# CPJKU/beat_this

Measured on AMD Instinct MI355X. Metric: audio-seconds processed/sec, higher is better.
Workload: dtype f32 activations, f16x3 products (3 x f16 MFMA on hi+lo operand halves, f32 accumulate); main-layer attention P.V: 2 x, probabilities as fp16 hi parts

## Files before the change

beat_this_amd/_lib.py:

```python
from __future__ import annotations

import ctypes as C
import os
import subprocess

import torch

PKG_DIR = os.path.dirname(os.path.abspath(__file__))
LIB_PATH = os.path.join(PKG_DIR, "libbeat_this_amd.so")
if os.environ.get("BT_DEV") == "1" and os.environ.get("BT_LIB_PATH"):
    LIB_PATH = os.environ["BT_LIB_PATH"]
SOURCES = ["gemm.hip", "gemm2.hip", "gemm3.hip", "gemm_mx8.hip", "attn.hip", "attn2.hip", "fused.hip", "fused2.hip", "qkv_front.hip", "frontend.hip", "logmel.hip",
           "tail.hip", "dbn.hip", "metrics.hip", "loss.hip", "data.hip", "train.hip", "optim.hip", "engine.hip"]
HEADERS = ["common.h", "chain.h", "kernels.h", "dropout.h", "train_mixed.inc", "attn_x3_loop.inc", "attn_hq2_loop.inc", os.path.join("..", "..", "include", "beat_this_amd.h")]

BT_OK, BT_ERR_ARG, BT_ERR_HIP, BT_ERR_WORKSPACE = 0, -1, -2, -3
ABI_VERSION = 600
PREC_F32, PREC_HALF, PREC_F32X3 = 0, 1, 3
OPT_X3_ATTN_P16, OPT_X3_GEMM_FP8, OPT_WS_GUARD = 1, 2, 3
MAX_LAYERS = 32
PROFILE_CATEGORIES = ["stem", "qkv_gemm", "attn_flash", "out_gemm", "ff1_gemm", "ff2_gemm", "conv_gemm",
                      "linear_gemm", "head", "ff_fused", "attn_freq_fused", "layer_tail"]

GEMM_EPI_STORE, GEMM_EPI_RESID, GEMM_EPI_QKV = 0, 1, 2
# ... 92 lines not shown
                ("residual", C.c_int32), ("sum_head", C.c_int32), ("reserved", C.c_int32), ("rope", C.c_void_p),
                ("gamma", C.c_void_p), ("w1", C.c_void_p), ("b1", C.c_void_p), ("w2", C.c_void_p), ("b2", C.c_void_p),
                ("w3", C.c_void_p), ("x", C.c_void_p), ("y", C.c_void_p), ("y2", C.c_void_p), ("save_o", C.c_void_p),
                ("save_lse", C.c_void_p), ("gy", C.c_void_p), ("gy2", C.c_void_p), ("gx", C.c_void_p), ("g_gamma", C.c_void_p),
                ("g_w1", C.c_void_p), ("g_b1", C.c_void_p), ("g_w2", C.c_void_p), ("g_b2", C.c_void_p), ("g_w3", C.c_void_p),
                ("ws", C.c_void_p), ("ws_bytes", C.c_size_t)]


class TrainDropout(C.Structure):
    _fields_ = [("p", C.c_float), ("reserved", C.c_uint32), ("seed", C.c_uint64), ("stream", C.c_uint64)]


class OptimTensor(C.Structure):
    _fields_ = [("param", C.c_void_p), ("offset", C.c_int64), ("numel", C.c_int64), ("group", C.c_int32), ("reserved", C.c_int32)]


class OptimChunk(C.Structure):
    _fields_ = [("tensor", C.c_int32), ("chunk", C.c_int32)]


class OptimGroup(C.Structure):
    _fields_ = [("decay", C.c_float), ("one_minus_beta1", C.c_float), ("beta2", C.c_float), ("one_minus_beta2", C.c_float),
                ("step_size", C.c_float), ("bias2_sqrt", C.c_float), ("eps", C.c_float), ("reserved", C.c_float)]


OPTIM_MAX_GROUPS = 8


class OptimHyper(C.Structure):
    _fields_ = [("n_groups", C.c_int32), ("zero_grads", C.c_int32), ("grad_scale", C.c_float), ("reserved", C.c_int32),
                ("g", OptimGroup * OPTIM_MAX_GROUPS)]


G3_FF1, G3_RESID, G3_QKV = 0, 1, 2
UNIT_STEM, UNIT_PARTIAL, UNIT_CONV, UNIT_LINEAR, UNIT_ATTN, UNIT_FF, UNIT_NORM, UNIT_FRONT_ATTN, UNIT_FRONT_FF = range(9)
TRAIN_UNIT_HEAD = 16
TRAIN_DW_ROWS, TRAIN_CS_ROWS, TRAIN_ATTN_BLOCK = 1024, 64, 64
DROP_ATTN_P, DROP_ATTN_OUT, DROP_FF_HIDDEN, DROP_FF_OUT = range(4)
OPTIM_CHUNK, OPTIM_NORM_SLICE = 4096, 4096

EXPORTS = {
    "bt_last_error": (C.c_char_p, []),
    "bt_version": (C.c_int, []),
    "bt_half_is_bf16": (C.c_int, []),
    "bt_struct_sizes": (None, [C.POINTER(C.c_int32)]),
    "bt_engine_create": (C.c_int, [C.POINTER(ModelDesc), C.POINTER(C.c_void_p)]),
    "bt_engine_destroy": (None, [C.c_void_p]),
    "bt_engine_set_option": (C.c_int, [C.c_void_p, C.c_int, C.c_int]),
    "bt_engine_get_option": (C.c_int, [C.c_void_p, C.c_int, C.POINTER(C.c_int)]),
    "bt_workspace_bytes": (C.c_size_t, [C.c_void_p, C.c_int, C.c_int, C.c_int]),
    "bt_workspace_regions": (C.c_int, [C.c_void_p, C.c_int, C.c_int, C.c_int, C.POINTER(C.c_int64), C.c_int]),
    "bt_forward": (C.c_int, [C.c_void_p, C.c_void_p, C.c_int, C.c_void_p, C.c_int, C.c_int, C.c_void_p, C.c_size_t,
                             C.c_void_p, C.c_void_p]),
    "bt_forward_stages": (C.c_int, [C.c_void_p, C.c_void_p, C.c_int, C.c_int, C.c_int, C.c_void_p, C.c_int, C.c_int, C.c_void_p,
                                    C.c_size_t, C.c_void_p, C.c_void_p, C.c_void_p]),
    "bt_forward_unit": (C.c_int, [C.c_void_p, C.c_void_p, C.c_int, C.c_int, C.c_int, C.c_void_p, C.c_void_p, C.c_int, C.c_int,
                                  C.c_void_p, C.c_size_t]),
    "bt_split_chunks": (C.c_int, [C.c_void_p, C.c_void_p, C.c_int64, C.c_void_p, C.c_int, C.c_int, C.c_void_p]),
    "bt_aggregate": (C.c_int, [C.c_void_p, C.c_void_p, C.c_void_p, C.c_void_p, C.c_int, C.c_int, C.c_int, C.c_int64,
                               C.c_void_p, C.c_void_p]),
    "bt_logmel": (C.c_int, [C.c_void_p, C.POINTER(LogmelTables), C.c_void_p, C.c_int64, C.c_void_p]),
    "bt_resample": (C.c_int, [C.c_void_p, C.c_void_p, C.c_int64, C.c_int, C.c_int, C.c_void_p, C.c_int, C.c_void_p,
                              C.c_int64]),
    "bt_peaks": (C.c_int, [C.c_void_p, C.c_void_p, C.c_int64, C.c_int, C.c_void_p, C.c_void_p]),
    "bt_deduplicate_peaks_host": (C.c_int, [C.c_void_p, C.c_int, C.c_double, C.c_void_p, C.POINTER(C.c_int32)]),
    "bt_postprocess_host": (C.c_int, [C.c_void_p, C.c_int, C.c_void_p, C.c_int, C.c_double, C.c_void_p,
                                      C.POINTER(C.c_int32), C.c_void_p, C.POINTER(C.c_int32)]),
    "bt_audio2beats_plan": (C.c_int, [C.c_void_p, C.c_int64, C.c_int, C.c_int, C.c_int, C.POINTER(A2BPlan)]),
    "bt_audio2beats_enqueue": (C.c_int, [C.c_void_p, C.c_void_p, C.c_int, C.POINTER(LogmelTables), C.c_void_p, C.c_int64, C.c_int, C.c_int,
                                         C.c_void_p, C.c_int, C.c_void_p, C.c_size_t, C.c_void_p, C.c_int]),
    "bt_profile_begin": (None, [C.c_void_p]),
    "bt_profile_end": (C.c_int, [C.c_void_p, C.c_void_p, C.c_void_p, C.c_int]),
    "bt_resample_batch": (C.c_int, [C.c_void_p, C.c_void_p, C.c_int, C.c_int64, C.c_int, C.c_int, C.c_void_p, C.c_int,
                                    C.c_void_p]),
    "bt_logmel_batch": (C.c_int, [C.c_void_p, C.POINTER(LogmelTables), C.c_void_p, C.c_int, C.c_int64, C.c_void_p]),
    "bt_split_chunks_batch": (C.c_int, [C.c_void_p, C.c_void_p, C.c_void_p, C.c_int, C.c_int, C.c_void_p]),
    "bt_aggregate_batch": (C.c_int, [C.c_void_p, C.c_void_p, C.c_void_p, C.c_void_p, C.c_void_p, C.c_int, C.c_int64,
                                     C.c_int, C.c_int, C.c_void_p, C.c_void_p]),
    "bt_peaks_batch": (C.c_int, [C.c_void_p, C.c_void_p, C.c_void_p, C.c_int, C.c_void_p, C.c_void_p]),
    "bt_peaks_host": (C.c_int, [C.c_void_p, C.c_int64, C.c_void_p, C.POINTER(C.c_int32)]),
    "bt_gemm": (C.c_int, [C.c_void_p, C.c_int, C.POINTER(GemmArgs)]),
    "bt_attention": (C.c_int, [C.c_void_p, C.c_int, C.POINTER(AttnArgs)]),
    "bt_gemm3": (C.c_int, [C.c_void_p, C.POINTER(Gemm3Args)]),
    "bt_gemm_mx8": (C.c_int, [C.c_void_p, C.c_void_p, C.c_void_p, C.c_void_p, C.c_void_p, C.c_void_p, C.c_int, C.c_int, C.c_int, C.c_int64]),
    "bt_attn_frag_blocks": (C.c_int, [C.c_int]),
    "bt_attention_frag": (C.c_int, [C.c_void_p, C.POINTER(AttnFragArgs)]),
    "bt_qkv_front": (C.c_int, [C.c_void_p, C.c_int, C.POINTER(PairWeights), C.c_void_p, C.c_void_p, C.c_int, C.c_int, C.c_int,
                               C.c_void_p, C.c_void_p, C.c_void_p, C.c_void_p, C.c_int]),
    "bt_outff_fused": (C.c_int, [C.c_void_p, C.c_int, C.POINTER(PairWeights), C.c_void_p, C.c_void_p, C.c_int64, C.c_void_p]),
    "bt_attnff_fused": (C.c_int, [C.c_void_p, C.c_int, C.POINTER(PairWeights), C.c_void_p, C.c_void_p, C.c_int64]),
    "bt_layer_tail": (C.c_int, [C.c_void_p, C.POINTER(PairWeights), C.c_int, C.c_void_p, C.c_void_p, C.c_int64, C.c_void_p,
                                C.c_void_p]),
    "bt_ff_fused": (C.c_int, [C.c_void_p, C.c_int, C.POINTER(PairWeights), C.c_void_p, C.c_int64]),
    "bt_dbn_tables": (C.c_int, [C.c_double, C.c_double, C.c_double, C.c_int, C.c_double, C.c_double, C.c_double, C.c_void_p,
                                C.c_int, C.c_void_p, C.POINTER(C.c_size_t)]),
    "bt_dbn_workspace_bytes": (C.c_size_t, [C.c_void_p, C.c_int, C.c_int64]),
    "bt_dbn_decode": (C.c_int, [C.c_void_p, C.c_void_p, C.c_void_p, C.c_void_p, C.c_int, C.c_void_p, C.c_int, C.c_int64,
                                C.c_void_p, C.c_void_p, C.c_size_t]),
    "bt_dbn_viterbi": (C.c_int, [C.c_void_p, C.c_void_p, C.c_void_p, C.c_int, C.c_void_p, C.c_int64, C.c_void_p, C.c_void_p,
                                 C.c_void_p, C.c_size_t]),
    "bt_dbn_viterbi_host": (C.c_int, [C.c_void_p, C.c_int, C.c_void_p, C.c_int64, C.c_void_p, C.c_void_p]),
    "bt_dbn_host": (C.c_int, [C.c_void_p, C.c_void_p, C.c_void_p, C.c_int64, C.c_void_p, C.POINTER(C.c_int32)]),
    "bt_dbn_host_act": (C.c_int, [C.c_void_p, C.c_void_p, C.c_int64, C.c_void_p, C.POINTER(C.c_int32)]),
    "bt_beat_metrics_workspace_bytes": (C.c_size_t, [C.c_int, C.c_int64, C.c_int64]),
    "bt_beat_metrics": (C.c_int, [C.c_void_p, C.c_void_p, C.c_void_p, C.c_void_p, C.c_void_p, C.c_int, C.c_double, C.c_double,
                                  C.c_double, C.c_double, C.c_double, C.c_void_p, C.c_size_t, C.c_void_p]),
    "bt_beat_metrics_host": (C.c_int, [C.c_void_p, C.c_void_p, C.c_void_p, C.c_void_p, C.c_int, C.c_double, C.c_double,
                                       C.c_double, C.c_double, C.c_double, C.c_void_p]),
    "bt_bce_loss_workspace_bytes": (C.c_size_t, [C.c_int, C.c_int64]),
    "bt_bce_loss": (C.c_int, [C.c_void_p, C.c_int, C.c_int, C.c_float, C.c_void_p, C.c_void_p, C.c_int, C.c_void_p, C.c_int,
                              C.c_void_p, C.c_int, C.c_void_p, C.c_int, C.c_int64, C.c_int64, C.c_void_p, C.c_size_t,
                              C.c_void_p, C.c_void_p, C.c_void_p, C.c_int, C.c_void_p, C.c_void_p]),
    "bt_bce_loss_backward": (C.c_int, [C.c_void_p, C.c_void_p, C.c_int64, C.c_void_p, C.c_int, C.c_int64, C.c_void_p, C.c_int]),
    "bt_bce_loss_host": (C.c_int, [C.c_int, C.c_int, C.c_float, C.c_void_p, C.c_int, C.c_void_p, C.c_int, C.c_void_p, C.c_int,
                                   C.c_void_p, C.c_int, C.c_void_p, C.c_void_p, C.c_void_p, C.c_void_p, C.c_void_p]),
    "bt_train_batch_struct_sizes": (None, [C.POINTER(C.c_int32)]),
    "bt_train_batch": (C.c_int, [C.c_void_p, C.c_void_p, C.c_int, C.c_int64, C.c_void_p, C.c_int, C.c_int, C.c_void_p, C.c_int,
                                 C.c_void_p, C.c_int, C.c_void_p, C.c_void_p, C.c_int64, C.c_double, C.c_void_p, C.c_int,
                                 C.c_void_p, C.c_void_p, C.c_void_p, C.c_void_p]),
    "bt_train_batch_host": (C.c_int, [C.c_void_p, C.c_int, C.c_int64, C.c_void_p, C.c_int, C.c_int, C.c_void_p, C.c_int,
                                      C.c_void_p, C.c_int, C.c_void_p, C.c_void_p, C.c_int64, C.c_double, C.c_void_p, C.c_int,
                                      C.c_void_p, C.c_void_p, C.c_void_p, C.c_void_p]),
    "bt_train_struct_sizes": (None, [C.POINTER(C.c_int32)]),
    "bt_train_workspace_bytes": (C.c_size_t, [C.c_int, C.c_int, C.c_int, C.c_int, C.c_int, C.c_int]),
    "bt_train_forward": (C.c_int, [C.c_void_p, C.c_int, C.POINTER(TrainArgs)]),
    "bt_train_backward": (C.c_int, [C.c_void_p, C.c_int, C.POINTER(TrainArgs)]),
    "bt_train_dropout_struct_sizes": (None, [C.POINTER(C.c_int32)]),
    "bt_train_workspace_bytes_dropout": (C.c_size_t, [C.c_int, C.c_int, C.c_int, C.c_int, C.c_int, C.c_int]),
    "bt_train_forward_dropout": (C.c_int, [C.c_void_p, C.c_int, C.POINTER(TrainArgs), C.POINTER(TrainDropout)]),
    "bt_train_backward_dropout": (C.c_int, [C.c_void_p, C.c_int, C.POINTER(TrainArgs), C.POINTER(TrainDropout)]),
    "bt_philox4x32_10_host": (None, [C.POINTER(C.c_uint32), C.POINTER(C.c_uint32), C.POINTER(C.c_uint32)]),
    "bt_dropout_mask_host": (C.c_int, [C.POINTER(TrainDropout), C.c_int, C.c_int, C.c_int, C.c_int, C.c_int, C.c_void_p]),
    "bt_train_workspace_bytes_mixed": (C.c_size_t, [C.c_int, C.c_int, C.c_int, C.c_int, C.c_int, C.c_int, C.c_int]),
    "bt_train_forward_mixed": (C.c_int, [C.c_void_p, C.c_int, C.POINTER(TrainArgs), C.POINTER(TrainDropout)]),
    "bt_train_backward_mixed": (C.c_int, [C.c_void_p, C.c_int, C.POINTER(TrainArgs), C.POINTER(TrainDropout)]),
    "bt_train_matmul_mixed": (C.c_int, [C.c_void_p, C.c_int, C.c_void_p, C.c_void_p, C.c_int, C.c_int, C.c_int, C.c_void_p]),
# ... 149 lines not shown
```

beat_this_amd/csrc/attn2.hip:

```cpp
#include <cstdlib>

#include "common.h"
#include "kernels.h"

namespace {

constexpr int KB = 4;
constexpr int BLK_BYTES = 2048;
constexpr int TILE_BYTES = KB * BLK_BYTES;
constexpr int SMEM_BYTES = 2 * 2 * TILE_BYTES + 16;

typedef const __attribute__((address_space(1))) void* gptr_t;
typedef __attribute__((address_space(3))) void* lptr_t;

DEVI int lane_id_fresh() {
  int z;
  asm volatile("s_mov_b32 %0, 0" : "=s"(z));
  return __builtin_amdgcn_mbcnt_hi(~0u, __builtin_amdgcn_mbcnt_lo(~0u, z));
}
DEVI unsigned pk2(float a, float b) {
  const hfx2 t = {(hf)a, (hf)b};
  return __builtin_bit_cast(unsigned, t);
}
DEVI void zero16(f32x16& a) {
// ... 905 lines not shown
template <int OUT>
DEVI void store_rows_x(const AttnFragP& p, const QStateX& st, float l_tot, int qi, bool okq, int sh, int g, float& amax) {
  const int seq = sh / p.heads, head = sh - seq * p.heads;
  const float gatev = okq ? p.gates[(long)sh * p.nbp * 32 + qi] : 0.f;
  const long orow = okq ? (long)(seq / p.o_div) * p.o_outer + (long)(seq % p.o_div) * p.o_inner + (long)qi * p.o_tok : 0;
  const float scale = okq ? gatev / l_tot : 0.f;
  if constexpr (OUT == 1) {
    float* op = reinterpret_cast<float*>(p.out) + orow * p.inner + head * 32 + 4 * g;
    if (okq) {
#pragma unroll
      for (int a = 0; a < 4; ++a)
        *reinterpret_cast<f32x4*>(op + 8 * a) = f32x4{st.acc[4 * a] * scale, st.acc[4 * a + 1] * scale,
                                                       st.acc[4 * a + 2] * scale, st.acc[4 * a + 3] * scale};
    }
  } else {
    hf* op = reinterpret_cast<hf*>(p.out) + orow * 2 * p.inner + head * 64 + 8 * g;
#pragma unroll
    for (int k = 0; k < 2; ++k) {
      unsigned xh[2], xl[2], yh[2], yl[2];
#pragma unroll
      for (int i = 0; i < 2; ++i) {
        const float a0 = st.acc[8 * k + 2 * i] * scale, a1 = st.acc[8 * k + 2 * i + 1] * scale;
        const float b0 = st.acc[8 * k + 4 + 2 * i] * scale, b1 = st.acc[8 * k + 4 + 2 * i + 1] * scale;
        split_hl4(a0, a1, b0, b1, xh[i], xl[i], yh[i], yl[i]);
        amax = fmaxf(amax, fmaxf(fmaxf(fabsf(a0), fabsf(a1)), fmaxf(fabsf(b0), fabsf(b1))));
        const float nan_probe = (a0 + a1) + (b0 + b1);
        amax = (okq && nan_probe != nan_probe) ? __builtin_inff() : amax;
      }
      auto h0 = __builtin_amdgcn_permlane32_swap(xh[0], yh[0], false, false);
      auto h1 = __builtin_amdgcn_permlane32_swap(xh[1], yh[1], false, false);
      if (p.out_f32 == 2) {
        const float s0 = st.acc[8 * k] * scale, s1 = st.acc[8 * k + 1] * scale, s2 = st.acc[8 * k + 2] * scale, s3 = st.acc[8 * k + 3] * scale;
        const float t0 = st.acc[8 * k + 4] * scale, t1 = st.acc[8 * k + 5] * scale, t2 = st.acc[8 * k + 6] * scale, t3 = st.acc[8 * k + 7] * scale;
        auto b8 = __builtin_amdgcn_permlane32_swap(pk4_f8(s0, s1, s2, s3), pk4_f8(t0, t1, t2, t3), false, false);
        auto c8 = __builtin_amdgcn_permlane32_swap(lo4_f8(s0, s1, s2, s3, xh[0], xh[1]), lo4_f8(t0, t1, t2, t3, yh[0], yh[1]), false, false);
        if (okq) {
          *reinterpret_cast<u32x4*>(op + 16 * k) = u32x4{h0[0], h1[0], h0[1], h1[1]};
          char* gb = reinterpret_cast<char*>(op) - 16 * g;
          *reinterpret_cast<u32x2*>(gb + 64 + 16 * k + 8 * g) = u32x2{b8[0], b8[1]};
          *reinterpret_cast<u32x2*>(gb + 96 + 16 * k + 8 * g) = u32x2{c8[0], c8[1]};
        }
      } else {
      auto l0 = __builtin_amdgcn_permlane32_swap(xl[0], yl[0], false, false);
      auto l1 = __builtin_amdgcn_permlane32_swap(xl[1], yl[1], false, false);
      if (okq) {
        *reinterpret_cast<u32x4*>(op + 16 * k) = u32x4{h0[0], h1[0], h0[1], h1[1]};
        *reinterpret_cast<u32x4*>(op + 32 + 16 * k) = u32x4{l0[0], l1[0], l0[1], l1[1]};
      }
      }
    }
  }
}

template <int QB, int OUT, int KBX, int MINW, bool P16>
__global__ __launch_bounds__(256, MINW) void attn_frag_x3_kernel(const AttnFragP p, int nqt, int sh_total) {
  constexpr int TILEX_BYTES = KBX * BLKX_BYTES;
  __shared__ __attribute__((aligned(16))) char smem[2 * 2 * TILEX_BYTES + 16];
  const int bid = blockIdx.x;
  const int idx = bid >> 3;
  const int sh = (idx / nqt) * 8 + (bid & 7);
  const int qt = idx % nqt;
  if (sh >= sh_total) return;
  const int tid = threadIdx.x, lane = tid & 63, wave = __builtin_amdgcn_readfirstlane(tid >> 6);
  const int g = lane >> 5, lr = lane & 31;
  const int L = p.L;
  const int nblk = (L + 31) >> 5;
  const long seq_off = (long)sh * p.nbp * BLKX_BYTES;
  const char* kseq = reinterpret_cast<const char*>(p.k) + seq_off;
  const char* vseq = reinterpret_cast<const char*>(p.v) + seq_off;
  QStateX st[QB];
  int qbi[QB];
  const int qb0 = (qt * 4 + wave) * QB;
#pragma unroll
  for (int j = 0; j < QB; ++j) {
    const int qbc = min(qb0 + j, nblk - 1);
    qbi[j] = qbc;
    const char* qblk = reinterpret_cast<const char*>(p.q) + seq_off + (long)qbc * BLKX_BYTES;
    st[j].q0 = *reinterpret_cast<const hfx8*>(qblk + ((2 * g) * 32 + lr) * 16);
    st[j].q1 = *reinterpret_cast<const hfx8*>(qblk + ((2 * g + 1) * 32 + lr) * 16);
    st[j].q0l = *reinterpret_cast<const hfx8*>(qblk + BLK_BYTES + ((2 * g) * 32 + lr) * 16);
    st[j].q1l = *reinterpret_cast<const hfx8*>(qblk + BLK_BYTES + ((2 * g + 1) * 32 + lr) * 16);
  }
  asm volatile("s_waitcnt vmcnt(0)" ::: "memory");
  __builtin_amdgcn_sched_barrier(0);
  const unsigned seq_bytes = (unsigned)p.nbp * BLKX_BYTES;
  const rsrc_t rk = __builtin_amdgcn_make_buffer_rsrc(const_cast<char*>(kseq), 0, seq_bytes, 0x00020000);
  const rsrc_t rv = __builtin_amdgcn_make_buffer_rsrc(const_cast<char*>(vseq), 0, seq_bytes, 0x00020000);
  float dmax[QB];
  diag_max_x<QB>(kseq, qbi, g, lr, st, L, dmax);
  attn_fast_x<QB, KBX, P16>(rk, rv, smem, tid, wave, lane, g, lr, st, L, nblk, dmax);
  auto lane_sum = [&](int j) { return P16 ? st[j].l4[0] : st[j].l; };
  float l_tot[QB];
  bool bad[QB];
#pragma unroll
  for (int j = 0; j < QB; ++j) {
    l_tot[j] = lane_sum(j) + __shfl_xor(lane_sum(j), 32);
    const bool valid = qb0 + j < nblk && (qb0 + j) * 32 + lr < L;
    bad[j] = valid && !(l_tot[j] < 65504.f);
    const unsigned long long bw = __ballot(bad[j]);
    if (lane == 0 && qb0 + j < nblk) p.fix_mask[(long)sh * p.nbp + qb0 + j] = (int)(unsigned)bw;
  }
#ifdef BT_DEV
  if (p.status && tid == 0) atomicAdd(p.status + 2, 1);
#endif

  float amax = 0.f;
#pragma unroll
  for (int j = 0; j < QB; ++j) {
    const int qi = (qb0 + j) * 32 + lr;
    store_rows_x<OUT>(p, st[j], l_tot[j], qi, qb0 + j < nblk && qi < L && !bad[j], sh, g, amax);
  }
  if (OUT == 0 && p.status && __any(!(amax <= (p.out_f32 == 2 ? HL8_ACT_MAX : 65504.f))) && lane == 0) atomicOr(p.status, 1);
}


#include "attn_x3_loop.inc"

template <int OUT, bool P16>
__global__ __launch_bounds__(256, 2) void attn_frag_x3q2_kernel(const AttnFragP p, int nqt, int sh_total) {
  constexpr int QB = 2, KBX = ATTN_X3Q2_KBX, NBUF = ATTN_X3Q2_NBUF;
  constexpr int TILEX_BYTES = KBX * BLKX_BYTES, BUF_BYTES = 2 * TILEX_BYTES;
  static_assert(KBX == 2 && NBUF == 4 && BUF_BYTES == 16384, "the generated loop is written for four 16 KB ring buffers");
  __shared__ __attribute__((aligned(16))) char smem[NBUF * BUF_BYTES + 16];
  const int bid = blockIdx.x;
  const int idx = bid >> 3;
  const int sh = (idx / nqt) * 8 + (bid & 7);
  const int qt = idx % nqt;
  if (sh >= sh_total) return;
  const int tid = threadIdx.x, lane = tid & 63, wave = __builtin_amdgcn_readfirstlane(tid >> 6);
  const int g = lane >> 5, lr = lane & 31;
  const int L = p.L;
  const int nblk = (L + 31) >> 5;
  const long seq_off = (long)sh * p.nbp * BLKX_BYTES;
  const char* kseq = reinterpret_cast<const char*>(p.k) + seq_off;
  const char* vseq = reinterpret_cast<const char*>(p.v) + seq_off;
  QStateX st[QB];
  const int qb0 = (qt * 4 + wave) * QB;
#ifndef BT_X3Q2_ONE
#define BT_X3Q2_ONE 1
#endif
  const bool one = BT_X3Q2_ONE && __builtin_amdgcn_readfirstlane((int)(qb0 + 1 >= nblk)) != 0;
  auto load_q = [&]() {
    const int ln = lane_id_fresh(), gg = ln >> 5, ll = ln & 31;
#pragma unroll
    for (int j = 0; j < QB; ++j) {
      if (j == 1 && one) {
        st[j].q0 = st[j].q1 = st[j].q0l = st[j].q1l = hfx8{0, 0, 0, 0, 0, 0, 0, 0};
        continue;
      }
      const int qbc = min(qb0 + j, nblk - 1);
      const char* qblk = reinterpret_cast<const char*>(p.q) + seq_off + (long)qbc * BLKX_BYTES;
      st[j].q0 = *reinterpret_cast<const hfx8*>(qblk + ((2 * gg) * 32 + ll) * 16);
      st[j].q1 = *reinterpret_cast<const hfx8*>(qblk + ((2 * gg + 1) * 32 + ll) * 16);
      st[j].q0l = *reinterpret_cast<const hfx8*>(qblk + BLK_BYTES + ((2 * gg) * 32 + ll) * 16);
      st[j].q1l = *reinterpret_cast<const hfx8*>(qblk + BLK_BYTES + ((2 * gg + 1) * 32 + ll) * 16);
    }
    asm volatile("s_waitcnt vmcnt(0)" ::: "memory");
    __builtin_amdgcn_sched_barrier(0);
  };
  load_q();
  float dmax[QB];
  {
    const int qbi[QB] = {min(qb0, nblk - 1), min(qb0 + 1, nblk - 1)};
    if (one) {
      diag_max_x<QB, 1>(kseq, qbi, g, lr, st, L, dmax);
      dmax[1] = -1e30f;
    } else {
      diag_max_x<QB>(kseq, qbi, g, lr, st, L, dmax);
    }
  }
  const unsigned seq_bytes = (unsigned)p.nbp * BLKX_BYTES;
  const rsrc_t rk = __builtin_amdgcn_make_buffer_rsrc(const_cast<char*>(kseq), 0, seq_bytes, 0x00020000);
  const rsrc_t rv = __builtin_amdgcn_make_buffer_rsrc(const_cast<char*>(vseq), 0, seq_bytes, 0x00020000);
  const int ntiles = (nblk + KBX - 1) / KBX;
  const bool partial = (L & 31) != 0;
  int nfull = nblk / KBX;
  if (partial && nfull * KBX == nblk) --nfull;
  nfull = __builtin_amdgcn_readfirstlane(nfull);
  auto stage_ring = [&](int tile) {
    char* kd = smem + (tile & (NBUF - 1)) * BUF_BYTES + wave * 1024;
    const int so = tile * TILEX_BYTES;
// ... 53 lines not shown
    asm volatile("s_waitcnt vmcnt(0)" ::: "memory");
    __syncthreads();
    if (nfull < ntiles) {
      load_q();
#pragma unroll
      for (int r = 0; r < 16; ++r) {
        st[0].negm[r] = nm0;
        st[1].negm[r] = nm1;
      }
      const int lane2 = lane_id_fresh(), g2 = lane2 >> 5, lr2 = lane2 & 31;
      const char* kb = smem + (nfull & (NBUF - 1)) * BUF_BYTES;
      const char* vb = kb + TILEX_BYTES;
      const int nb = nblk - nfull * KBX;
      for (int c = 0; c < nb; ++c) {
        const int blk = nfull * KBX + c;
        const KFragX kf = ld_kx(kb + c * BLKX_BYTES, g2, lr2);
        const VFragX vf = ld_vx(vb + c * BLKX_BYTES, lane2);
        f32x16 sc[QB];
        if (one) {
          score_x<true, QB, 1>(kf, st, sc);
          if (partial && blk == nblk - 1) finish_x<false, true, QB, true, P16, 1>(sc, vf, g2, st, blk * 32, L);
          else finish_x<false, false, QB, true, P16, 1>(sc, vf, g2, st, blk * 32, L);
        } else {
          score_x<true, QB>(kf, st, sc);
          if (partial && blk == nblk - 1) finish_x<false, true, QB, true, P16>(sc, vf, g2, st, blk * 32, L);
          else finish_x<false, false, QB, true, P16>(sc, vf, g2, st, blk * 32, L);
        }
      }
      __syncthreads();
    }
  };
  stage_ring(0);
  stage_ring(1);
  stage_ring(2);
  asm volatile("s_waitcnt vmcnt(8)" ::: "memory");
  __syncthreads();
  if (one) {
    ref_max_x<QB, 1>(smem, g, lr, st, L, nblk, dmax);
    zero16(st[1].negm);
  } else {
    ref_max_x<QB>(smem, g, lr, st, L, nblk, dmax);
  }
  fast_pass();
  auto lane_sum = [&](int j) { return P16 ? st[j].l4[0] : st[j].l; };
  const int laneE = lane_id_fresh(), gE = laneE >> 5, lrE = laneE & 31;
  float l_tot[QB];
  bool bad[QB];
#pragma unroll
  for (int j = 0; j < QB; ++j) {
    l_tot[j] = lane_sum(j) + __shfl_xor(lane_sum(j), 32);
    const bool valid = qb0 + j < nblk && (qb0 + j) * 32 + lrE < L;
    bad[j] = valid && !(l_tot[j] < 65504.f);
    const unsigned long long bw = __ballot(bad[j]);
    if (laneE == 0 && qb0 + j < nblk) p.fix_mask[(long)sh * p.nbp + qb0 + j] = (int)(unsigned)bw;
  }
#ifdef BT_DEV
  if (p.status && tid == 0) atomicAdd(p.status + 2, 1);
#endif

  const int seq = sh / p.heads, head = sh - seq * p.heads;
  float amax = 0.f;
#pragma unroll
  for (int j = 0; j < QB; ++j) {
    if (j == 1 && one) continue;
    const int qi = (qb0 + j) * 32 + lrE;
    const bool okq = qb0 + j < nblk && qi < L && !bad[j];
    const float gatev = okq ? p.gates[(long)sh * p.nbp * 32 + qi] : 0.f;
    const long orow = okq ? (long)(seq / p.o_div) * p.o_outer + (long)(seq % p.o_div) * p.o_inner + (long)qi * p.o_tok : 0;
    const float scale = okq ? gatev / l_tot[j] : 0.f;
    if constexpr (OUT == 1) {
      float* op = reinterpret_cast<float*>(p.out) + orow * p.inner + head * 32 + 4 * gE;
      if (okq) {
#pragma unroll
        for (int a = 0; a < 4; ++a)
          *reinterpret_cast<f32x4*>(op + 8 * a) = f32x4{st[j].acc[4 * a] * scale, st[j].acc[4 * a + 1] * scale,
                                                         st[j].acc[4 * a + 2] * scale, st[j].acc[4 * a + 3] * scale};
      }
    } else {
      hf* op = reinterpret_cast<hf*>(p.out) + orow * 2 * p.inner + head * 64 + 8 * gE;
#pragma unroll
      for (int k = 0; k < 2; ++k) {
        unsigned xh[2], xl[2], yh[2], yl[2];
#pragma unroll
        for (int i = 0; i < 2; ++i) {
          const float a0 = st[j].acc[8 * k + 2 * i] * scale, a1 = st[j].acc[8 * k + 2 * i + 1] * scale;
          const float b0 = st[j].acc[8 * k + 4 + 2 * i] * scale, b1 = st[j].acc[8 * k + 4 + 2 * i + 1] * scale;
          split_hl4(a0, a1, b0, b1, xh[i], xl[i], yh[i], yl[i]);
          amax = fmaxf(amax, fmaxf(fmaxf(fabsf(a0), fabsf(a1)), fmaxf(fabsf(b0), fabsf(b1))));
        }
        auto h0 = __builtin_amdgcn_permlane32_swap(xh[0], yh[0], false, false);
        auto h1 = __builtin_amdgcn_permlane32_swap(xh[1], yh[1], false, false);
        if (p.out_f32 == 2) {
          const float s0 = st[j].acc[8 * k] * scale, s1 = st[j].acc[8 * k + 1] * scale, s2 = st[j].acc[8 * k + 2] * scale, s3 = st[j].acc[8 * k + 3] * scale;
          const float t0 = st[j].acc[8 * k + 4] * scale, t1 = st[j].acc[8 * k + 5] * scale, t2 = st[j].acc[8 * k + 6] * scale, t3 = st[j].acc[8 * k + 7] * scale;
          auto b8 = __builtin_amdgcn_permlane32_swap(pk4_f8(s0, s1, s2, s3), pk4_f8(t0, t1, t2, t3), false, false);
          auto c8 = __builtin_amdgcn_permlane32_swap(lo4_f8(s0, s1, s2, s3, xh[0], xh[1]), lo4_f8(t0, t1, t2, t3, yh[0], yh[1]), false, false);
          if (okq) {
            *reinterpret_cast<u32x4*>(op + 16 * k) = u32x4{h0[0], h1[0], h0[1], h1[1]};
            char* gb = reinterpret_cast<char*>(op) - 16 * gE;
            *reinterpret_cast<u32x2*>(gb + 64 + 16 * k + 8 * gE) = u32x2{b8[0], b8[1]};
            *reinterpret_cast<u32x2*>(gb + 96 + 16 * k + 8 * gE) = u32x2{c8[0], c8[1]};
          }
        } else {
        auto l0 = __builtin_amdgcn_permlane32_swap(xl[0], yl[0], false, false);
        auto l1 = __builtin_amdgcn_permlane32_swap(xl[1], yl[1], false, false);
        if (okq) {
          *reinterpret_cast<u32x4*>(op + 16 * k) = u32x4{h0[0], h1[0], h0[1], h1[1]};
// ... 251 lines not shown
```

beat_this_amd/csrc/common.h:

```cpp
#pragma once
#include <hip/hip_runtime.h>
#include <stdint.h>

#ifdef BT_HALF_BF16
typedef __bf16 hf;
#define BT_HALF_IS_BF16 1
#define MFMA32_H(a, b, c) __builtin_amdgcn_mfma_f32_32x32x16_bf16(a, b, c, 0, 0, 0)
#else
typedef _Float16 hf;
#define BT_HALF_IS_BF16 0
#define MFMA32_H(a, b, c) __builtin_amdgcn_mfma_f32_32x32x16_f16(a, b, c, 0, 0, 0)
#endif
typedef __attribute__((ext_vector_type(8))) hf hfx8;
typedef __attribute__((ext_vector_type(4))) hf hfx4;
typedef __attribute__((ext_vector_type(2))) hf hfx2;
typedef __attribute__((ext_vector_type(16))) float f32x16;
typedef __attribute__((ext_vector_type(4))) float f32x4;
typedef __attribute__((ext_vector_type(2))) float f32x2;

#define DEVI __device__ __forceinline__

template <typename T> struct Frag;
template <> struct Frag<float> { f32x4 v[4]; };
template <> struct Frag<hf> { hfx8 v[2]; };
struct hl { hf hi, lo; };
template <> struct Frag<hl> { hfx8 v[4]; };
template <typename T> struct OpScale { static constexpr float ACT = 1.f, PW = 1.f, PA = 1.f; };
template <> struct OpScale<hl> { static constexpr float ACT = 32.f, PW = 1.f / (32.f * 64.f), PA = 1.f / (32.f * 32.f); };

template <typename T> struct Tile { static constexpr int PITCH = 32 * (int)sizeof(T) + 16; };

template <typename T> DEVI Frag<T> ld_frag(const char* row_ptr, int g);
template <> DEVI Frag<float> ld_frag<float>(const char* row_ptr, int g) {
  Frag<float> f;
  const f32x4* p = reinterpret_cast<const f32x4*>(row_ptr + g * 64);
#pragma unroll
  for (int i = 0; i < 4; ++i) f.v[i] = p[i];
  return f;
}
template <> DEVI Frag<hf> ld_frag<hf>(const char* row_ptr, int g) {
  Frag<hf> f;
  const hfx8* p = reinterpret_cast<const hfx8*>(row_ptr + g * 32);
  f.v[0] = p[0];
  f.v[1] = p[1];
  return f;
}

DEVI void mma32(f32x16& acc, const Frag<float>& a, const Frag<float>& b) {
#pragma unroll
  for (int i = 0; i < 4; ++i)
#pragma unroll
    for (int j = 0; j < 4; ++j) acc = __builtin_amdgcn_mfma_f32_32x32x2f32(a.v[i][j], b.v[i][j], acc, 0, 0, 0);
}
DEVI void mma32(f32x16& acc, const Frag<hf>& a, const Frag<hf>& b) {
  acc = MFMA32_H(a.v[0], b.v[0], acc);
  acc = MFMA32_H(a.v[1], b.v[1], acc);
}
DEVI void mma32(f32x16& acc, const Frag<hl>& a, const Frag<hl>& b) {
  acc = MFMA32_H(a.v[2], b.v[0], acc);
  acc = MFMA32_H(a.v[3], b.v[1], acc);
  acc = MFMA32_H(a.v[0], b.v[2], acc);
  acc = MFMA32_H(a.v[1], b.v[3], acc);
  acc = MFMA32_H(a.v[0], b.v[0], acc);
  acc = MFMA32_H(a.v[1], b.v[1], acc);
}

DEVI int crow(int r, int g) { return (r & 3) + 8 * (r >> 2) + 4 * g; }

DEVI float gelu_erf(float x) {
  const float t = __builtin_amdgcn_rcpf(fmaf(0.2316418882f, fabsf(x), 1.0f));
  float p = fmaf(1.061405429f, t, -1.453152027f);
  p = fmaf(p, t, 1.421413741f);
  p = fmaf(p, t, -0.284496736f);
  p = fmaf(p, t, 0.254829592f);
  const float e = 0.5f * p * t * __builtin_amdgcn_exp2f(-0.7213475204f * x * x);
  return x * (x < 0.f ? e : 1.0f - e);
}
DEVI float gelu_tanh(float x) {
  const float x2 = fminf(x * x, 49.0f);
  const float pol = fmaf(fmaf(x2, 0.001014263f, -0.106775716f), x2, -2.3011212f);
  const float e = __builtin_amdgcn_exp2f(x * pol);
  return x * __builtin_amdgcn_rcpf(1.0f + e);
}
template <typename T> DEVI float gelu_t(float x);
template <> DEVI float gelu_t<float>(float x) { return gelu_erf(x); }
template <> DEVI float gelu_t<hf>(float x) { return gelu_tanh(x); }
template <> DEVI float gelu_t<hl>(float x) { return gelu_erf(x); }
DEVI float sigmoidf(float x) { return 1.0f / (1.0f + __expf(-x)); }

template <typename T> DEVI T from_f32(float x);
template <> DEVI float from_f32<float>(float x) { return x; }
template <> DEVI hf from_f32<hf>(float x) { return (hf)x; }

DEVI void split_hl4(float a0, float b0, float a1, float b1, unsigned& h0, unsigned& l0, unsigned& h1, unsigned& l1) {
  const float m1 = -1.0f;
  asm("s_nop 0\n\t"
      "v_cvt_pk_f16_f32 %0, %4, %5\n\t"
      "v_cvt_pk_f16_f32 %2, %6, %7\n\t"
      "v_fma_mixlo_f16 %1, %0, %8, %4 op_sel:[0,0,0] op_sel_hi:[1,0,0]\n\t"
      "v_fma_mixlo_f16 %3, %2, %8, %6 op_sel:[0,0,0] op_sel_hi:[1,0,0]\n\t"
      "v_fma_mixhi_f16 %1, %0, %8, %5 op_sel:[1,0,0] op_sel_hi:[1,0,0]\n\t"
      "v_fma_mixhi_f16 %3, %2, %8, %7 op_sel:[1,0,0] op_sel_hi:[1,0,0]\n\t"
      "s_nop 0"
      : "=&v"(h0), "=&v"(l0), "=&v"(h1), "=&v"(l1)
      : "v"(a0), "v"(b0), "v"(a1), "v"(b1), "s"(m1));
}
DEVI void split_hl(float a, float b, unsigned& whi, unsigned& wlo) {
  const float m1 = -1.0f;
  asm("s_nop 0\n\t"
      "v_cvt_pk_f16_f32 %0, %2, %3\n\t"
      "v_fma_mixlo_f16 %1, %0, %4, %2 op_sel:[0,0,0] op_sel_hi:[1,0,0]\n\t"
      "s_nop 0\n\t"
      "v_fma_mixhi_f16 %1, %0, %4, %3 op_sel:[1,0,0] op_sel_hi:[1,0,0]\n\t"
      "s_nop 0"
      : "=&v"(whi), "=&v"(wlo)
      : "v"(a), "v"(b), "s"(m1));
}

#ifndef BT_HL8_ACT_EXP
#define BT_HL8_ACT_EXP 3
// ... 28 lines not shown
```

beat_this_amd/csrc/engine.hip:

```cpp
#include <algorithm>
#include <cmath>
#include <cstddef>
#include <cstdio>
#include <cstring>
#include <mutex>
#include <string>
#include <vector>

#include "../../include/beat_this_amd.h"
#include "common.h"
#include "kernels.h"


static thread_local std::string g_err;
static int bt_set_error(int code, const std::string& msg) {
  g_err = msg;
  return code;
}
int bt_set_error_external(int code, const char* msg) { return bt_set_error(code, msg); }

namespace prof {
struct Rec { int cat; hipEvent_t a, b; };
struct State { bool on = false; std::vector<Rec> recs; };
struct Scope {
// ... 89 lines not shown
  p.spect = spect; p.x = x; p.bn1_scale = d.bn1_scale; p.bn1_shift = d.bn1_shift;
  p.w = d.stem_w; p.bias = d.stem_b; p.B = B; p.T = T;
  return p;
}

GemmP conv_params(const bt_model_desc& d, int blk, int wp, const float* in, void* out, int B, int T, bool out_f32) {
  const int C = 32 << blk, F = 32 >> blk;
  GemmP g;
  memset(&g, 0, sizeof g);
  g.A = in; g.W = d.conv_w[blk][wp]; g.M = B * T * (F / 2); g.N = 2 * C; g.K = 6 * C;
  g.epi = GEMM_EPI_STORE; g.flags = GEMM_F_CONV | GEMM_F_A_F32 | GEMM_F_BIAS | GEMM_F_GELU | (out_f32 ? GEMM_F_OUT_F32 : 0);
  g.bias = d.conv_b[blk]; g.out = out; g.ldo = 2 * C;
  g.conv_C2 = 2 * C; g.conv_T = T; g.conv_F = F / 2;
  return g;
}

Gemm3P conv3_params(const bt_model_desc& d, const Workspace& ws, int blk, int B, int T, bool x3, bool out_half) {
  const int C = 32 << blk, F = 32 >> blk;
  float* out = front_x(ws, blk + 1);
  Gemm3P g;
  memset(&g, 0, sizeof g);
  g.A = ws.hid; g.lda = 2 * C; g.M = B * T * (F / 2); g.K = 6 * C; g.N = 2 * C;
  g.W = x3 ? d.conv_w_x3[blk] : d.conv_w[blk][BT_PREC_HALF];
  g.epi = G3_RESID; g.no_resid = 1; g.gelu = 1; g.bias = d.conv_b[blk]; g.ldx = 2 * C;
  g.conv_C2 = 2 * C; g.conv_T = T; g.conv_F = F / 2; g.x3 = x3; g.status = ws.status;
  g.x = out_half ? nullptr : out; g.xb = out_half ? (void*)out : nullptr;
  return g;
}

GemmP linear_params(const bt_model_desc& d, int wp, const float* in, float* out, void* xb, float* ssq_out, int B, int T) {
  GemmP g;
  memset(&g, 0, sizeof g);
  g.A = in; g.lda = 1024; g.W = d.lin_w[wp]; g.M = B * T; g.N = d.transformer_dim; g.K = 1024;
  g.epi = GEMM_EPI_STORE; g.flags = GEMM_F_A_F32 | GEMM_F_BIAS | GEMM_F_OUT_F32;
  g.bias = d.lin_b; g.out = out; g.ldo = d.transformer_dim; g.xb = xb; g.ssq_out = ssq_out;
  return g;
}

Gemm3P linear3_params(const bt_model_desc& d, const Workspace& ws, int B, int T, bool x3, bool out_f8) {
  const int D = d.transformer_dim;
  Gemm3P g;
  memset(&g, 0, sizeof g);
  g.A = front_x(ws, 3); g.lda = 1024; g.M = B * T; g.K = 1024; g.W = x3 ? d.lin_w_x3 : d.lin_w[BT_PREC_HALF]; g.N = D;
  g.epi = G3_RESID; g.no_resid = 1; g.bias = d.lin_b; g.x = ws.xm; g.ldx = D; g.xb = ws.xmb; g.ssq_out = ws.ssq[0];
  g.x3 = x3 ? 1 | (out_f8 ? G3_X3_OUT_F8 : 0) : 0; g.status = ws.status;
  return g;
}

HeadP head_params(const bt_model_desc& d, const float* x, const float* w, int prenorm, float* beat, float* downbeat, int M,
                  int* status) {
  HeadP p;
  p.x = x; p.w = w; p.b0 = d.head_b[0]; p.b1 = d.head_b[1];
  p.beat = beat; p.downbeat = downbeat; p.M = M; p.D = d.transformer_dim; p.sum_head = d.sum_head; p.prenorm = prenorm;
  p.status = status;
  return p;
}

template <class P>
void attn_rows(P& a, int B, int T, int F) {
  a.n_seq = B * F; a.L = T; a.o_div = F; a.o_outer = (long)T * F; a.o_inner = F > 1 ? 1 : 0; a.o_tok = F;
}

struct PairRoute {
  bool ff_fused;
  bool outff;
  bool split;
  bool time_frag;
};

struct FragLayer {
  bool qkv8;
  bool out8;
  bool ff8;
  bool next8;
  bool tail;
  bool shadow_dead;
};

enum { LAYERS_GENERIC, LAYERS_FRAG_HALF, LAYERS_FRAG_X3 };

struct Route {
  bool x3;
  int fp;
  int gp, wp;
  int x3_attn, x3_attn_front;
  bool half_shadow;
  int layers;
  struct Block { PairRoute freq, time; bool conv3; bool x_dead; } blk[3];
  bool lin3, lin_f8;
  struct Layer { PairRoute pair; FragLayer frag; } layer[BT_MAX_LAYERS];
};

#ifndef BT_SKIP_DEAD_STORES
#define BT_SKIP_DEAD_STORES 1
#endif
Route plan_route(const bt_engine& e, int B, int T, int prec, int first, int last, const Workspace& ws) {
  const bt_model_desc& d = e.d;
  const int D = d.transformer_dim;
  Route r;
  r.x3 = prec == BT_PREC_F32X3;
  r.fp = r.x3 ? BT_PREC_F32 : prec;
  r.gp = prec;
  r.wp = r.x3 ? BT_PREC_HALF : prec;
  r.x3_attn = r.x3 ? 4 | ((e.x3_attn_p16 == 1 || e.x3_attn_p16 == 2) ? BT_X3_P16 : 0) : 0;
  r.x3_attn_front = r.x3 ? 4 | (e.x3_attn_p16 >= 2 ? BT_X3_P16 : 0) : 0;
  auto pair = [&](const bt_pair_weights& w) {
    PairRoute p;
    p.ff_fused = w.dim <= 128 && w.w_ff_frag[r.fp];
    p.outff = p.ff_fused && w.w_outff_frag[r.fp] && w.w_attnff_frag[r.fp];
    p.split = r.x3 && w.w_outff_frag_x3 && w.w_attnff_frag_x3;
    p.time_frag = r.x3 ? p.outff && p.split && w.w_qkv_frag_x3 : p.ff_fused && r.fp == BT_PREC_HALF && w.w_qkv_frag;
    return p;
  };

  r.half_shadow = prec == BT_PREC_HALF && D >= 128 && D % 64 == 0;
  const long wide = (long)B * T * d.ff_mult * D;
  bool frag_x3 = r.x3 && D >= 128 && D % 128 == 0 && wide * 4 < 0x7fffffffL;
  for (int l = 0; frag_x3 && l < d.n_layers; ++l)
    frag_x3 = d.layers[l].w_qkvg_x3 && d.layers[l].w_out_x3 && d.layers[l].w_ff1_x3 && d.layers[l].w_ff2_x3;
  const bool frag_half = r.half_shadow && D % 128 == 0 && wide * 2 < 0x7fffffffL;
  r.layers = frag_x3 ? LAYERS_FRAG_X3 : frag_half ? LAYERS_FRAG_HALF : LAYERS_GENERIC;

  const bool lin3_fits = (frag_half || (frag_x3 && d.lin_w_x3)) && gemm3_supported(linear3_params(d, ws, B, T, frag_x3, false));
  for (int blk = 0; blk < 3; ++blk) {
    Route::Block& rb = r.blk[blk];
    rb.freq = pair(d.front[blk][0]);
    rb.time = pair(d.front[blk][1]);
    const Gemm3P cg = conv3_params(d, ws, blk, B, T, frag_x3, blk == 2 && lin3_fits);
    rb.conv3 = d.partial_transformers && rb.time.outff && (frag_x3 ? rb.time.split : frag_half) && cg.N >= 128 && cg.W &&
               gemm3_supported(cg);
    rb.x_dead = BT_SKIP_DEAD_STORES && rb.conv3 && frag_x3;
  }
  r.lin3 = lin3_fits && (!frag_x3 || r.blk[2].conv3);
  r.lin_f8 = r.lin3 && frag_x3 && e.x3_gemm_fp8 >= 2 && d.n_layers > 0 && d.layers[0].w_qkvg_f8;

  for (int l = 0; l < d.n_layers; ++l) {
    const bt_pair_weights& w = d.layers[l];
    FragLayer& f = r.layer[l].frag;
    r.layer[l].pair = pair(w);
    f.qkv8 = l == 0 ? first == 0 && r.lin_f8 : r.layer[l - 1].frag.next8;
    f.out8 = frag_x3 && e.x3_gemm_fp8 >= 2 && w.w_out_f8;
    f.ff8 = frag_x3 && e.x3_gemm_fp8 >= 1 && w.w_ff1_f8 && w.w_ff2_f8;
    f.next8 = frag_x3 && e.x3_gemm_fp8 >= 2 && l + 1 < d.n_layers && d.layers[l + 1].w_qkvg_f8 && w.w_ff2_f8;
    f.tail = frag_half && w.w_tail_frag && layer_tail_supported(D, d.ff_mult * D);
    f.shadow_dead = BT_SKIP_DEAD_STORES && frag_x3 && last == 2 && l == d.n_layers - 1;
  }
  return r;
}

#define CHECK_RC(what)                                                         \
  if (_rc != 0) {                                                              \
    char buf[160];                                                             \
    snprintf(buf, sizeof buf, "%s failed (code %d: %s)", what, _rc,            \
             _rc > 0 ? hipGetErrorString((hipError_t)_rc) : "bad arguments");  \
    return bt_set_error(_rc > 0 ? BT_ERR_HIP : BT_ERR_ARG, buf);               \
  }
#define LAUNCH(expr, what) \
  do { int _rc = (expr); CHECK_RC(what) } while (0)
#define LAUNCH_CAT(cat, st, expr, what) \
  do { int _rc; { prof::Scope _ps(pf, cat, st); _rc = (expr); } CHECK_RC(what) } while (0)


int check_rows(long M) {
  return M > 0x7fffffffL ? bt_set_error(BT_ERR_ARG, "batch too large for one forward call") : BT_OK;
}

int out_proj(prof::State* pf, const bt_pair_weights& pw, const Route& r, float* x, void* xs, const Workspace& ws, long M,
             hipStream_t s) {
  const int C = pw.dim;
  GemmP g;
  memset(&g, 0, sizeof g);
  g.A = ws.ao; g.lda = C; g.W = pw.w_out[r.wp]; g.M = (int)M; g.N = C; g.K = C;
  g.epi = GEMM_EPI_RESID; g.flags = 0; g.x = x; g.ldx = C; g.xb = xs;
  LAUNCH_CAT(CAT_OUT, s, launch_gemm(g, r.gp, s), "out-proj gemm");
  return BT_OK;
}

int qkv_attn(prof::State* pf, const bt_pair_weights& pw, const Route& r, const float* rope, float* x, void* xs,
             const Workspace& ws, int B, int T, int F, hipStream_t s) {
  const int C = pw.dim, H = pw.heads;
  GemmP g;
  memset(&g, 0, sizeof g);
  g.A = xs ? xs : (const void*)x; g.lda = C; g.W = pw.w_qkvg[r.wp]; g.M = B * T * F; g.N = 3 * C + H; g.K = C;
  g.epi = GEMM_EPI_QKV; g.flags = GEMM_F_RMS | (xs ? 0 : GEMM_F_A_F32) | (F > 1 ? GEMM_F_ROWMAP : 0);
  g.bias = pw.b_gates; g.out = ws.qkv; g.ldo = 3 * C; g.gates = ws.gates; g.inner = C; g.heads = H;
  g.rope = rope; g.map_T = T; g.map_F = F; g.pdiv = F; g.pmod = T;
  LAUNCH_CAT(CAT_QKV, s, launch_gemm(g, r.gp, s), "qkv gemm");
  AttnP a;
  memset(&a, 0, sizeof a);
  a.qkv = ws.qkv; a.ld = 3 * C; a.gates = ws.gates; a.out = ws.ao; a.heads = H; a.inner = C;
  attn_rows(a, B, T, F);
  LAUNCH_CAT(CAT_ATTN_FLASH, s, launch_attn_flash(a, r.gp, s), F > 1 ? "time attention" : "attention");
  return BT_OK;
}

int ff_half(prof::State* pf, const bt_pair_weights& pw, const PairRoute& pr, const Route& r, float* x, void* xs,
            const Workspace& ws, long M, int ff_mult, hipStream_t s) {
  const int C = pw.dim, HID = ff_mult * C;
// ... 35 lines not shown
  FusedAttnFFP f;
  f.x = x; f.M = M; f.C = pw.dim; f.b_gates = pw.b_gates; f.rope = rope;
  f.wfrag = pr.split ? pw.w_attnff_frag_x3 : pw.w_attnff_frag[r.fp]; f.b1 = pw.b_ff1; f.b2 = pw.b_ff2;
  LAUNCH_CAT(CAT_ATTN_FREQ_FUSED, s, launch_attnff_fused(f, pr.split ? BT_PREC_F32X3 : r.fp, s),
             "fused frequency attention + feed-forward");
  return BT_OK;
}

int time_half(prof::State* pf, const bt_pair_weights& pw, const PairRoute& pr, const Route& r, const float* rope, float* x,
              const Workspace& ws, int B, int T, int F, void* shadow, bool shadow_only, hipStream_t s) {
  const long M = (long)B * T * F;
  if (int rc = check_rows(M)) return rc;
  if (pr.time_frag) {
    QkvFrontP qp;
    memset(&qp, 0, sizeof qp);
    qp.x = x; qp.B = B; qp.T = T; qp.F = F; qp.C = pw.dim; qp.wfrag = r.x3 ? pw.w_qkv_frag_x3 : pw.w_qkv_frag;
    qp.b_gates = pw.b_gates; qp.rope = rope;
    qp.q = ws.qf; qp.k = ws.kf; qp.v = ws.vf; qp.gates = ws.gates_h; qp.nbp = ws.nbp;
    qp.x3 = r.x3; qp.status = ws.status;
    LAUNCH_CAT(CAT_QKV, s, launch_qkv_front(qp, s), "frontend qkv projection");
    AttnFragP a;
    memset(&a, 0, sizeof a);
    a.q = ws.qf; a.k = ws.kf; a.v = ws.vf; a.gates = ws.gates_h; a.out = ws.ao; a.heads = pw.heads; a.inner = pw.dim;
    a.nbp = ws.nbp; attn_rows(a, B, T, F);
    a.x3 = r.x3_attn_front; a.out_f32 = 1; a.status = ws.status; a.fix_mask = ws.fix_mask;
    LAUNCH_CAT(CAT_ATTN_FLASH, s, launch_attn_frag(a, s), "time attention");
  } else if (int rc = qkv_attn(pf, pw, r, rope, x, nullptr, ws, B, T, F, s)) {
    return rc;
  }
  if (pr.outff) {
    FusedOutFFP f;
    f.x = x; f.M = M; f.C = pw.dim; f.ao = ws.ao; f.wfrag = pr.split ? pw.w_outff_frag_x3 : pw.w_outff_frag[r.fp];
    f.b1 = pw.b_ff1; f.b2 = pw.b_ff2; f.xb = shadow; f.abl = 0; f.shadow_only = shadow && shadow_only && pr.split;
    LAUNCH_CAT(CAT_FF_FUSED, s, launch_outff_fused(f, pr.split ? BT_PREC_F32X3 : r.fp, s), "fused out-projection + feed-forward");
    return BT_OK;
  }
  if (int rc = out_proj(pf, pw, r, x, nullptr, ws, M, s)) return rc;
  return ff_half(pf, pw, pr, r, x, nullptr, ws, M, 4, s);
}

int frag_layer(prof::State* pf, const bt_pair_weights& pw, const FragLayer& f, const Route& r, const float* rope,
               const Workspace& ws, int B, int T, int ff_mult, hipStream_t s) {
  const int D = pw.dim, H = pw.heads, HID = ff_mult * D;
  const int M = B * T;
  const int parts = D / 64;
  int* status = r.x3 ? ws.status : nullptr;
  auto w = [&](const void* const* half, const void* hl32, const void* hl8, bool f8) { return !r.x3 ? half[BT_PREC_HALF] : f8 ? hl8 : hl32; };
  Gemm3P g;
  memset(&g, 0, sizeof g);
  g.A = ws.xmb; g.lda = D; g.M = M; g.K = D; g.W = w(pw.w_qkvg, pw.w_qkvg_x3, pw.w_qkvg_f8, f.qkv8); g.N = 3 * D + H; g.epi = G3_QKV;
  g.ssq_in = ws.ssq[0]; g.ssq_parts = parts; g.x3 = r.x3 | (f.qkv8 ? G3_X3_F8 : 0); g.status = status;
  g.n_seq = B; g.L = T; g.nblk = (T + 31) / 32; g.nbp = ws.nbp; g.heads = H; g.inner = D; g.rope = rope;
  g.qf = ws.qf; g.kf = ws.kf; g.vf = ws.vf; g.gates = ws.gates_h; g.b_gates = pw.b_gates;
  LAUNCH_CAT(CAT_QKV, s, launch_gemm3(g, s), r.x3 ? "qkv gemm (hi + lo)" : "qkv gemm");
  AttnFragP a;
  memset(&a, 0, sizeof a);
  a.q = ws.qf; a.k = ws.kf; a.v = ws.vf; a.gates = ws.gates_h; a.out = ws.ao; a.heads = H; a.inner = D; a.nbp = ws.nbp;
  attn_rows(a, B, T, 1);
  a.x3 = r.x3_attn; a.out_f32 = f.out8 ? 2 : 0; a.status = status; a.fix_mask = ws.fix_mask;
  LAUNCH_CAT(CAT_ATTN_FLASH, s, launch_attn_frag(a, s), r.x3 ? "attention (hi + lo)" : "attention");
  if (f.tail) {
    LayerTailP t;
    t.x = ws.xm; t.M = M; t.C = D; t.hidden = HID; t.ao = ws.ao; t.wfrag = pw.w_tail_frag; t.b1 = pw.b_ff1; t.b2 = pw.b_ff2;
    t.xb = ws.xmb; t.ssq_out = ws.ssq[0];
    LAUNCH_CAT(CAT_LAYER_TAIL, s, launch_layer_tail(t, s), "layer tail (out-projection + feed-forward)");
    return BT_OK;
  }
  memset(&g, 0, sizeof g);
  g.A = ws.ao; g.lda = D; g.M = M; g.K = D; g.W = w(pw.w_out, pw.w_out_x3, pw.w_out_f8, f.out8); g.N = D; g.epi = G3_RESID;
  g.x3 = r.x3 | (f.out8 ? G3_X3_F8 : 0) | (f.ff8 ? G3_X3_OUT_F8 : 0); g.status = status;
  g.x = ws.xm; g.ldx = D; g.xb = ws.xmb; g.ssq_out = ws.ssq[1];
  LAUNCH_CAT(CAT_OUT, s, launch_gemm3(g, s), r.x3 ? "out-proj gemm (hi + lo)" : "out-proj gemm");
  memset(&g, 0, sizeof g);
  g.A = ws.xmb; g.lda = D; g.M = M; g.K = D; g.W = w(pw.w_ff1, pw.w_ff1_x3, pw.w_ff1_f8, f.ff8); g.N = HID; g.epi = G3_FF1;
  g.x3 = r.x3 | (f.ff8 ? G3_X3_F8 | G3_X3_OUT_F8 : 0); g.status = status;
  g.bias = pw.b_ff1; g.ssq_in = ws.ssq[1]; g.ssq_parts = parts; g.out = ws.hid; g.ldo = HID;
  LAUNCH_CAT(CAT_FF1, s, launch_gemm3(g, s), r.x3 ? "ff1 gemm (hi + lo)" : "ff1 gemm");
  memset(&g, 0, sizeof g);
  g.A = ws.hid; g.lda = HID; g.M = M; g.K = HID; g.W = w(pw.w_ff2, pw.w_ff2_x3, pw.w_ff2_f8, f.ff8); g.N = D; g.epi = G3_RESID;
  g.x3 = r.x3 | (f.ff8 ? G3_X3_F8 : 0) | (f.next8 ? G3_X3_OUT_F8 : 0); g.status = status;
  g.bias = pw.b_ff2; g.x = ws.xm; g.ldx = D; g.xb = f.shadow_dead ? nullptr : ws.xmb; g.ssq_out = f.shadow_dead ? nullptr : ws.ssq[0];
  LAUNCH_CAT(CAT_FF2, s, launch_gemm3(g, s), r.x3 ? "ff2 gemm (hi + lo)" : "ff2 gemm");
  return BT_OK;
}

int frontend(prof::State* pf, const bt_model_desc& d, const Route& r, const float* spect, const Workspace& ws, int B, int T,
             hipStream_t s) {
  const StemP sp = stem_params(d, spect, front_x(ws, 0), B, T);
  LAUNCH_CAT(CAT_STEM, s, launch_stem(sp, s), "stem");
  for (int blk = 0; blk < 3; ++blk) {
    const Route::Block& rb = r.blk[blk];
    float* x = front_x(ws, blk);
    if (d.partial_transformers) {
      if (int rc = freq_half(pf, d.front[blk][0], rb.freq, r, d.rope, x, B, T, 32 >> blk, s)) return rc;
      if (int rc = time_half(pf, d.front[blk][1], rb.time, r, d.rope, x, ws, B, T, 32 >> blk, rb.conv3 ? ws.hid : nullptr, rb.x_dead, s))
        return rc;
    }
    if (rb.conv3) {
      const Gemm3P g = conv3_params(d, ws, blk, B, T, r.layers == LAYERS_FRAG_X3, blk == 2 && r.lin3);
      LAUNCH_CAT(CAT_CONV, s, launch_gemm3(g, s), "frontend conv gemm");
    } else {
      const GemmP g = conv_params(d, blk, r.wp, x, front_x(ws, blk + 1), B, T, !(blk == 2 && r.lin3));
      LAUNCH_CAT(CAT_CONV, s, launch_gemm(g, r.gp, s), "frontend conv gemm");
    }
  }
  if (r.lin3) {
    const Gemm3P g = linear3_params(d, ws, B, T, r.layers == LAYERS_FRAG_X3, r.lin_f8);
    LAUNCH_CAT(CAT_LINEAR, s, launch_gemm3(g, s), "frontend linear gemm");
    return BT_OK;
  }
  const GemmP g = linear_params(d, r.wp, front_x(ws, 3), ws.xm, r.half_shadow ? ws.xmb : nullptr,
                                r.layers == LAYERS_FRAG_HALF ? ws.ssq[0] : nullptr, B, T);
  LAUNCH_CAT(CAT_LINEAR, s, launch_gemm(g, r.gp, s), "frontend linear gemm");
  if (r.layers == LAYERS_FRAG_X3)
    LAUNCH_CAT(CAT_LINEAR, s, launch_shadow_ssq(ws.xm, ws.xmb, ws.ssq[0], (long)B * T, d.transformer_dim, s, 1), "hl32 shadow of the residual stream");
  return BT_OK;
}

}

extern "C" {

const char* bt_last_error(void) { return g_err.c_str(); }
int bt_version(void) { return BT_ABI_VERSION; }
int bt_half_is_bf16(void) { return BT_HALF_IS_BF16; }
void bt_struct_sizes(int32_t* out) {
  out[0] = (int32_t)sizeof(bt_pair_weights); out[1] = (int32_t)sizeof(bt_model_desc);
  out[2] = (int32_t)sizeof(bt_logmel_tables); out[3] = (int32_t)sizeof(bt_gemm_args);
  out[4] = (int32_t)sizeof(bt_attn_args); out[5] = (int32_t)offsetof(bt_model_desc, layers);
  out[6] = (int32_t)offsetof(bt_model_desc, rope);
  out[7] = (int32_t)sizeof(bt_attn_frag_args);
  out[8] = (int32_t)sizeof(bt_gemm3_args);
}

// ... 6 lines not shown
  e->d = *desc;
  *out = e;
  return BT_OK;
}
static void drop_graphs(bt_engine* e) {
  for (auto& g : e->graphs) (void)hipGraphExecDestroy(g.exec);
  e->graphs.clear();
  e->warm.clear();
}
void bt_engine_destroy(bt_engine* e) {
  if (!e) return;
  for (auto& r : e->prof.recs) { (void)hipEventDestroy(r.a); (void)hipEventDestroy(r.b); }
  drop_graphs(e);
  if (e->cap_stream) (void)hipStreamDestroy(e->cap_stream);
  delete e;
}

int bt_engine_set_option(bt_engine* e, int option, int value) {
  if (!e) return bt_set_error(BT_ERR_ARG, "null argument");
  std::lock_guard<std::mutex> lock(e->mu);
  if (option == BT_OPT_X3_ATTN_P16 && value >= 0 && value <= 3) { if (e->x3_attn_p16 != value) drop_graphs(e); e->x3_attn_p16 = value; return BT_OK; }
  if (option == BT_OPT_X3_GEMM_FP8 && value >= 0 && value <= 2) { if (e->x3_gemm_fp8 != value) drop_graphs(e); e->x3_gemm_fp8 = value; return BT_OK; }
  if (option == BT_OPT_WS_GUARD && value >= 0 && value % 256 == 0) { if (e->ws_guard != value) drop_graphs(e); e->ws_guard = value; return BT_OK; }
  return bt_set_error(BT_ERR_ARG, "unknown engine option / value");
}
int bt_engine_get_option(const bt_engine* e, int option, int* value) {
  if (!e || !value) return bt_set_error(BT_ERR_ARG, "null argument");
  if (option == BT_OPT_X3_ATTN_P16) { *value = e->x3_attn_p16; return BT_OK; }
  if (option == BT_OPT_X3_GEMM_FP8) { *value = e->x3_gemm_fp8; return BT_OK; }
  if (option == BT_OPT_WS_GUARD) { *value = e->ws_guard; return BT_OK; }
  return bt_set_error(BT_ERR_ARG, "unknown engine option");
}

size_t bt_workspace_bytes(const bt_engine* e, int B, int T, int prec) {
  if (!e || B <= 0 || T <= 0) return 0;
  return carve(nullptr, B, T, e->d.transformer_dim, e->d.ff_mult, prec, (size_t)e->ws_guard).total;
}

int bt_workspace_regions(const bt_engine* e, int B, int T, int prec, int64_t* begin_end, int max) {
  if (!e || B <= 0 || T <= 0 || max < 0 || (max > 0 && !begin_end)) return bt_set_error(BT_ERR_ARG, "bad argument to bt_workspace_regions");
  if (prec != BT_PREC_F32 && prec != BT_PREC_HALF && prec != BT_PREC_F32X3) return bt_set_error(BT_ERR_ARG, "unknown precision");
  std::vector<int64_t> r;
  carve(nullptr, B, T, e->d.transformer_dim, e->d.ff_mult, prec, (size_t)e->ws_guard, &r);
  const int n = (int)(r.size() / 2);
  for (int i = 0; i < std::min(n, max); ++i) { begin_end[2 * i] = r[2 * i]; begin_end[2 * i + 1] = r[2 * i + 1]; }
  return n;
}

int bt_forward(bt_engine* e, void* stream, int prec, const float* d_spect, int B, int T, void* d_ws, size_t ws_bytes,
               float* d_beat, float* d_downbeat) {
  return bt_forward_stages(e, stream, prec, 0, 2, d_spect, B, T, d_ws, ws_bytes, nullptr, d_beat, d_downbeat);
}

int bt_forward_stages(bt_engine* e, void* stream, int prec, int first, int last, const float* d_spect, int B, int T, void* d_ws,
                      size_t ws_bytes, float* d_out, float* d_beat, float* d_downbeat) {
  if (!e || !d_spect || !d_ws) return bt_set_error(BT_ERR_ARG, "null argument");
  if (first < 0 || last > 2 || first > last) return bt_set_error(BT_ERR_ARG, "stages: need 0 <= first <= last <= 2");
  if (last == 2 ? (!d_beat || !d_downbeat) : !d_out) return bt_set_error(BT_ERR_ARG, "null output");
  const int max_T = e->d.rope_len > 0 ? e->d.rope_len : 1536;
  if (B <= 0 || T <= 0 || T > max_T)
    return bt_set_error(BT_ERR_ARG, "need B >= 1 and 1 <= T <= " + std::to_string(max_T) + " (bt_model_desc.rope_len: rows of the rotary table)");
  if (prec != BT_PREC_F32 && prec != BT_PREC_HALF && prec != BT_PREC_F32X3)
    return bt_set_error(BT_ERR_ARG, "unknown precision");
  const bt_model_desc& d = e->d;
  prof::State* pf = &e->prof;
  const int D = d.transformer_dim;
  const Workspace ws = carve((char*)d_ws, B, T, D, d.ff_mult, prec, (size_t)e->ws_guard);
  if (ws.total > ws_bytes) return bt_set_error(BT_ERR_WORKSPACE, "workspace too small");
  if (prec == BT_PREC_F32X3 && BT_HALF_IS_BF16) return bt_set_error(BT_ERR_ARG, "BT_PREC_F32X3 needs an IEEE fp16 build");
  const Route r = plan_route(*e, B, T, prec, first, last, ws);
  hipStream_t s = (hipStream_t)stream;
  if (r.x3) LAUNCH(launch_clear_words(ws.status, 1, s), "clearing the range flag");
  int* status = r.x3 ? ws.status : nullptr;

  const size_t xm_bytes = (size_t)B * T * D * 4;
  if (first == 2) {
    if (!d.head_w_raw) return bt_set_error(BT_ERR_ARG, "stage entry at task_heads needs head_w_raw");
    const HeadP hp = head_params(d, d_spect, d.head_w_raw, 1, d_beat, d_downbeat, B * T, nullptr);
    LAUNCH_CAT(CAT_HEAD, s, launch_head(hp, s), "head");
    return BT_OK;
  }
  if (first == 1) {
    if (hipMemcpyAsync(ws.xm, d_spect, xm_bytes, hipMemcpyDeviceToDevice, s) != hipSuccess)
      return bt_set_error(BT_ERR_HIP, "copy of the stage input");
    if (r.half_shadow)
      LAUNCH_CAT(CAT_LINEAR, s, launch_shadow_ssq(ws.xm, ws.xmb, r.layers == LAYERS_FRAG_HALF ? ws.ssq[0] : nullptr, (long)B * T, D, s), "stage entry");
    if (r.layers == LAYERS_FRAG_X3) LAUNCH_CAT(CAT_LINEAR, s, launch_shadow_ssq(ws.xm, ws.xmb, ws.ssq[0], (long)B * T, D, s, 1), "stage entry");
  }
  if (first == 0)
    if (int rc = frontend(pf, d, r, d_spect, ws, B, T, s)) return rc;
  if (last == 0) {
    if (hipMemcpyAsync(d_out, ws.xm, xm_bytes, hipMemcpyDeviceToDevice, s) != hipSuccess)
      return bt_set_error(BT_ERR_HIP, "copy of the stage output");
    if (r.x3) LAUNCH_CAT(CAT_HEAD, s, launch_finite_rows(ws.xm, (long)B * T, D, ws.status, s), "range check of the stage output");
    return BT_OK;
  }
  for (int l = 0; l < d.n_layers; ++l) {
    const Route::Layer& rl = r.layer[l];
    const int rc = r.layers == LAYERS_GENERIC
                       ? generic_layer(pf, d.layers[l], rl.pair, r, d.rope, ws.xm, r.half_shadow ? ws.xmb : nullptr, ws, B, T,
                                       d.ff_mult, true, true, s)
                       : frag_layer(pf, d.layers[l], rl.frag, r, d.rope, ws, B, T, d.ff_mult, s);
    if (rc) return rc;
  }
  if (last == 1) {
    if (!d.norm_out_g) return bt_set_error(BT_ERR_ARG, "stage exit after transformer_blocks needs norm_out_g");
    LAUNCH_CAT(CAT_HEAD, s, launch_norm_out(ws.xm, d.norm_out_g, d_out, (long)B * T, D, s, status), "final norm");
    return BT_OK;
  }
  const HeadP hp = head_params(d, ws.xm, d.head_w, 0, d_beat, d_downbeat, B * T, status);
  LAUNCH_CAT(CAT_HEAD, s, launch_head(hp, s), "head");
  return BT_OK;
}

int bt_forward_unit(bt_engine* e, void* stream, int prec, int unit, int index, const float* d_in, float* d_out, int B, int T,
                    void* d_ws, size_t ws_bytes) {
  if (!e || !d_in || !d_out || !d_ws) return bt_set_error(BT_ERR_ARG, "null argument");
  const bt_model_desc& d = e->d;
  const int max_T = d.rope_len > 0 ? d.rope_len : 1536;
  if (B <= 0 || T <= 0 || T > max_T) return bt_set_error(BT_ERR_ARG, "need B >= 1 and 1 <= T <= bt_model_desc.rope_len");
  if (prec == BT_PREC_F32X3) prec = BT_PREC_F32;
  if (prec != BT_PREC_F32 && prec != BT_PREC_HALF) return bt_set_error(BT_ERR_ARG, "unknown precision");
  prof::State* pf = &e->prof;
  const int D = d.transformer_dim;
  const Workspace ws = carve((char*)d_ws, B, T, D, d.ff_mult, prec, (size_t)e->ws_guard);
  if (ws.total > ws_bytes) return bt_set_error(BT_ERR_WORKSPACE, "workspace too small");
  const Route r = plan_route(*e, B, T, prec, 0, 0, ws);
  hipStream_t s = (hipStream_t)stream;
  const bool block_unit = unit == BT_UNIT_PARTIAL || unit == BT_UNIT_CONV;
  const bool layer_unit = unit == BT_UNIT_ATTN || unit == BT_UNIT_FF;
  const bool leaf_unit = unit == BT_UNIT_FRONT_ATTN || unit == BT_UNIT_FRONT_FF;
  if (leaf_unit && (index < 0 || index > 5 || !d.partial_transformers)) return bt_set_error(BT_ERR_ARG, "partial-transformer leaf index out of range");
  if (block_unit && (index < 0 || index > 2)) return bt_set_error(BT_ERR_ARG, "frontend block index out of range");
  if (layer_unit && (index < 0 || index >= d.n_layers)) return bt_set_error(BT_ERR_ARG, "layer index out of range");
  auto copy_in = [&](size_t bytes) -> int {
    if (d_in != d_out && hipMemcpyAsync(d_out, d_in, bytes, hipMemcpyDeviceToDevice, s) != hipSuccess)
      return bt_set_error(BT_ERR_HIP, "copy of the unit's input");
    return BT_OK;
  };
  switch (unit) {
    case BT_UNIT_STEM: {
      const StemP sp = stem_params(d, d_in, d_out, B, T);
      LAUNCH_CAT(CAT_STEM, s, launch_stem(sp, s), "stem");
      return BT_OK;
    }
    case BT_UNIT_PARTIAL: {
      if (!d.partial_transformers) return bt_set_error(BT_ERR_ARG, "this model has no partial transformers");
      const Route::Block& rb = r.blk[index];
      if (int rc = copy_in((size_t)B * T * 1024 * 4)) return rc;
      if (int rc = freq_half(pf, d.front[index][0], rb.freq, r, d.rope, d_out, B, T, 32 >> index, s)) return rc;
      return time_half(pf, d.front[index][1], rb.time, r, d.rope, d_out, ws, B, T, 32 >> index, nullptr, false, s);
    }
    case BT_UNIT_CONV: {
      const GemmP g = conv_params(d, index, r.wp, d_in, d_out, B, T, true);
      LAUNCH_CAT(CAT_CONV, s, launch_gemm(g, r.gp, s), "frontend conv gemm");
      return BT_OK;
    }
    case BT_UNIT_LINEAR: {
      const GemmP g = linear_params(d, r.wp, d_in, d_out, nullptr, nullptr, B, T);
      LAUNCH_CAT(CAT_LINEAR, s, launch_gemm(g, r.gp, s), "frontend linear gemm");
      return BT_OK;
    }
    case BT_UNIT_ATTN:
// ... 194 lines not shown
  plan->n22 = n22; plan->n_frames = n;
  plan->T = n > fresh ? chunk : (int)n + 2 * border;
  plan->B = (int)((n + fresh - 1) / fresh);
  plan->result_words = 2 * n + 3;
  size_t off = 0;
  auto take = [&](size_t bytes) { size_t o = off; off += align_up(bytes, 256); return o; };
  plan->forward_bytes = bt_workspace_bytes(e, plan->B, plan->T, prec);
  plan->off_forward = take(plan->forward_bytes);
  plan->off_chunks = take((size_t)plan->B * plan->T * 128 * 4);
  plan->off_chunk_logits = take((size_t)2 * plan->B * plan->T * 4);
  plan->off_wave22 = take(up == down ? 0 : (size_t)n22 * 4);
  plan->off_spect = take((size_t)n * 128 * 4);
  plan->off_logits = take((size_t)2 * n * 4);
  plan->off_result = take((size_t)plan->result_words * 4);
  plan->ws_bytes = off;
  return BT_OK;
}

int bt_audio2beats_enqueue(bt_engine* e, void* stream, int prec, const bt_logmel_tables* t, const float* d_audio, int64_t n_in,
                           int up, int down, const float* d_filter, int half_len, void* d_ws, size_t ws_bytes, int32_t* h_result,
                           int use_graph) {
  if (!e || !t || !d_audio || !d_ws || !h_result) return bt_set_error(BT_ERR_ARG, "null argument");
  if (up != down && (!d_filter || half_len < 0)) return bt_set_error(BT_ERR_ARG, "resampling needs the polyphase filter");
  bt_a2b_plan pl;
  if (int rc = bt_audio2beats_plan(e, n_in, up, down, prec, &pl)) return rc;
  if (pl.ws_bytes > ws_bytes) return bt_set_error(BT_ERR_WORKSPACE, "workspace too small (bt_audio2beats_plan)");
  std::lock_guard<std::mutex> lock(e->mu);
  const int max_T = e->d.rope_len > 0 ? e->d.rope_len : 1536;
  if (pl.T > max_T) return bt_set_error(BT_ERR_ARG, "chunk longer than the rotary table");
  hipStream_t s = (hipStream_t)stream;
  char* ws = (char*)d_ws;
  float* wave22 = (float*)(ws + pl.off_wave22);
  float* spect = (float*)(ws + pl.off_spect);
  float* chunks = (float*)(ws + pl.off_chunks);
  float* cb = (float*)(ws + pl.off_chunk_logits);
  float* cd = cb + (size_t)pl.B * pl.T;
  float* beat = (float*)(ws + pl.off_logits);
  float* downb = beat + pl.n_frames;
  int32_t* res = (int32_t*)(ws + pl.off_result);
  void* fws = ws + pl.off_forward;
  const int border = 6;
  const float* a22 = d_audio;
  if (up != down) {
    const bt_span_t one{d_audio, (long)n_in, 0, (long)pl.n22};
    LAUNCH(launch_resample(one, nullptr, 1, (long)pl.n22, up, down, d_filter, half_len, wave22, s), "resample");
    a22 = wave22;
  }
  LogmelP lp;
  fill_logmel(lp, t, spect);
  lp.one = bt_span_t{a22, (long)pl.n22, 0, (long)pl.n_frames};
  lp.tracks = nullptr; lp.n_tracks = 1; lp.max_frames = (long)pl.n_frames;
  LAUNCH(launch_logmel(lp, s), "logmel");
  LAUNCH(launch_split(spect, (long)pl.n_frames, nullptr, nullptr, pl.B, pl.T, chunks, s, border), "split");
  const int warm_key = prec << 8 | pl.B;
  const bool graphable = use_graph && pl.T == 1500 && pl.B <= 16 && !e->prof.on &&
                         std::find(e->warm.begin(), e->warm.end(), warm_key) != e->warm.end();
  FwdGraph* g = nullptr;
  if (graphable) {
    for (auto& c : e->graphs)
      if (c.B == pl.B && c.T == pl.T && c.prec == prec && c.ws == d_ws) g = &c;
    if (!g) {
      hipGraph_t graph = nullptr;
      if (!e->cap_stream && hipStreamCreateWithFlags(&e->cap_stream, hipStreamNonBlocking) != hipSuccess) e->cap_stream = nullptr;
      if (e->cap_stream && hipStreamBeginCapture(e->cap_stream, hipStreamCaptureModeThreadLocal) == hipSuccess) {
        const int rc = bt_forward_stages(e, e->cap_stream, prec, 0, 2, chunks, pl.B, pl.T, fws, pl.forward_bytes, nullptr, cb, cd);
        const hipError_t he = hipStreamEndCapture(e->cap_stream, &graph);
        hipGraphExec_t exec = nullptr;
        if (rc == BT_OK && he == hipSuccess && graph && hipGraphInstantiate(&exec, graph, nullptr, nullptr, 0) == hipSuccess) {
          if (e->graphs.size() >= 8) {
            size_t old = 0;
            for (size_t i = 1; i < e->graphs.size(); ++i)
              if (e->graphs[i].stamp < e->graphs[old].stamp) old = i;
            (void)hipGraphExecDestroy(e->graphs[old].exec);
            e->graphs.erase(e->graphs.begin() + old);
          }
          e->graphs.push_back(FwdGraph{pl.B, pl.T, prec, d_ws, exec, 0});
          g = &e->graphs.back();
        }
        if (graph) (void)hipGraphDestroy(graph);
        (void)hipGetLastError();
      }
    }
  }
  if (g) {
    g->stamp = ++e->graph_clock;
    if (hipGraphLaunch(g->exec, s) != hipSuccess) return bt_set_error(BT_ERR_HIP, "replay of the captured forward");
  } else {
    if (int rc = bt_forward_stages(e, s, prec, 0, 2, chunks, pl.B, pl.T, fws, pl.forward_bytes, nullptr, cb, cd)) return rc;
    if (pl.T == 1500 && pl.B <= 16 && std::find(e->warm.begin(), e->warm.end(), warm_key) == e->warm.end()) e->warm.push_back(warm_key);
  }
  LAUNCH(launch_aggregate(cb, cd, nullptr, nullptr, nullptr, 1, pl.B, pl.T, border, (long)pl.n_frames, beat, downb, s), "aggregate");
  LAUNCH(launch_peaks(beat, (long)pl.n_frames, nullptr, 2, res, res + 2 * pl.n_frames, s), "peaks");
  if (prec == BT_PREC_F32X3) {
    if (hipMemcpyAsync(res + 2 * pl.n_frames + 2, fws, 4, hipMemcpyDeviceToDevice, s) != hipSuccess)
      return bt_set_error(BT_ERR_HIP, "copy of the range flag");
  } else if (hipMemsetAsync(res + 2 * pl.n_frames + 2, 0, 4, s) != hipSuccess) {
    return bt_set_error(BT_ERR_HIP, "clearing the range flag");
  }
  if (hipMemcpyAsync(h_result, res, (size_t)pl.result_words * 4, hipMemcpyDeviceToHost, s) != hipSuccess)
    return bt_set_error(BT_ERR_HIP, "device-to-host copy of the result");
  return BT_OK;
}

void bt_profile_begin(bt_engine* e) {
  if (!e) return;
  for (auto& r : e->prof.recs) { (void)hipEventDestroy(r.a); (void)hipEventDestroy(r.b); }
  e->prof.recs.clear();
  e->prof.on = true;
}

int bt_profile_end(bt_engine* e, double* ms_by_category, int32_t* launches_by_category, int n_categories) {
  if (!e) return bt_set_error(BT_ERR_ARG, "null engine");
  e->prof.on = false;
  if (!ms_by_category || !launches_by_category || n_categories < CAT_COUNT)
    return bt_set_error(BT_ERR_ARG, "need room for BT_PROFILE_CATEGORIES entries");
  for (int i = 0; i < n_categories; ++i) { ms_by_category[i] = 0.0; launches_by_category[i] = 0; }
  for (auto& r : e->prof.recs) {
    hipError_t e = hipEventSynchronize(r.b);
    float ms = 0.f;
    if (e == hipSuccess) e = hipEventElapsedTime(&ms, r.a, r.b);
    if (e != hipSuccess) return bt_set_error(BT_ERR_HIP, hipGetErrorString(e));
    ms_by_category[r.cat] += ms;
    launches_by_category[r.cat] += 1;
    (void)hipEventDestroy(r.a); (void)hipEventDestroy(r.b);
  }
  e->prof.recs.clear();
  return BT_OK;
}

int bt_ff_fused(void* stream, int prec, const bt_pair_weights* w, float* d_x, int64_t M) {
  if (!w || !d_x || M <= 0 || w->dim > 128 || !w->w_ff_frag[prec]) return bt_set_error(BT_ERR_ARG, "bad argument to bt_ff_fused");
  FusedFFP ff;
  ff.x = d_x; ff.M = M; ff.C = w->dim; ff.wfrag = w->w_ff_frag[prec]; ff.b1 = w->b_ff1; ff.b2 = w->b_ff2;
  ff.xb = nullptr;
  LAUNCH(launch_ff_fused(ff, prec, (hipStream_t)stream), "fused feed-forward");
  return BT_OK;
}

int bt_gemm(void* stream, int prec, const bt_gemm_args* a) {
  if (!a) return bt_set_error(BT_ERR_ARG, "null argument");
  GemmP g;
// ... 1 lines not shown
  g.A = a->A; g.lda = a->lda; g.W = a->W; g.M = a->M; g.N = a->N; g.K = a->K; g.epi = a->epi; g.flags = a->flags;
  g.bias = a->bias; g.out = a->out; g.ldo = a->ldo; g.x = a->x; g.ldx = a->ldx;
  g.conv_C2 = a->conv_C2; g.conv_T = a->conv_T; g.conv_F = a->conv_F;
  g.gates = a->gates; g.inner = a->inner; g.heads = a->heads; g.rope = a->rope;
  g.pdiv = a->pdiv; g.pmod = a->pmod; g.map_T = a->map_T; g.map_F = a->map_F;
  LAUNCH(launch_gemm(g, prec, (hipStream_t)stream), "gemm");
  return BT_OK;
}

int bt_attention(void* stream, int prec, const bt_attn_args* a) {
  if (!a) return bt_set_error(BT_ERR_ARG, "null argument");
  AttnP p;
  memset(&p, 0, sizeof p);
  p.qkv = a->qkv; p.ld = a->ld; p.gates = a->gates; p.out = a->out; p.n_seq = a->n_seq; p.L = a->L;
  p.heads = a->heads; p.inner = a->inner; p.o_div = a->o_div; p.o_outer = a->o_outer; p.o_inner = a->o_inner;
  p.o_tok = a->o_tok;
  LAUNCH(launch_attn_flash(p, prec, (hipStream_t)stream), "attention (flash)");
  return BT_OK;
}

int bt_outff_fused(void* stream, int prec, const bt_pair_weights* w, const void* d_ao, float* d_x, int64_t M, void* d_xb) {
  if (prec != BT_PREC_F32 && prec != BT_PREC_HALF && prec != BT_PREC_F32X3) return bt_set_error(BT_ERR_ARG, "unknown precision");
  const void* wf = !w ? nullptr : prec == BT_PREC_F32X3 ? w->w_outff_frag_x3 : w->w_outff_frag[prec];
  if (!w || !d_ao || !d_x || M <= 0 || w->dim > 128 || !wf) return bt_set_error(BT_ERR_ARG, "bad argument to bt_outff_fused");
  FusedOutFFP f;
  f.x = d_x; f.M = M; f.C = w->dim; f.ao = d_ao; f.wfrag = wf; f.b1 = w->b_ff1; f.b2 = w->b_ff2;
  f.xb = prec == BT_PREC_F32 ? nullptr : d_xb; f.abl = 0; f.shadow_only = 0;
  LAUNCH(launch_outff_fused(f, prec, (hipStream_t)stream), "fused out-projection + feed-forward");
  return BT_OK;
}

int bt_attnff_fused(void* stream, int prec, const bt_pair_weights* w, const float* d_rope, float* d_x, int64_t M) {
  if (prec != BT_PREC_F32 && prec != BT_PREC_HALF && prec != BT_PREC_F32X3) return bt_set_error(BT_ERR_ARG, "unknown precision");
  const void* wf = !w ? nullptr : prec == BT_PREC_F32X3 ? w->w_attnff_frag_x3 : w->w_attnff_frag[prec];
  if (!w || !d_x || !d_rope || M <= 0 || w->dim > 128 || !wf) return bt_set_error(BT_ERR_ARG, "bad argument to bt_attnff_fused");
  FusedAttnFFP f;
  f.x = d_x; f.M = M; f.C = w->dim; f.b_gates = w->b_gates; f.rope = d_rope; f.wfrag = wf;
  f.b1 = w->b_ff1; f.b2 = w->b_ff2;
  LAUNCH(launch_attnff_fused(f, prec, (hipStream_t)stream), "fused frequency attention + feed-forward");
  return BT_OK;
}

int bt_layer_tail(void* stream, const bt_pair_weights* w, int hidden, const void* d_ao, float* d_x, int64_t M, void* d_xb,
                  float* d_ssq_out) {
  if (!w || !w->w_tail_frag || !d_ao || !d_x || M <= 0 || !layer_tail_supported(w->dim, hidden))
    return bt_set_error(BT_ERR_ARG, "bad argument to bt_layer_tail");
  LayerTailP t;
  t.x = d_x; t.M = M; t.C = w->dim; t.hidden = hidden; t.ao = d_ao; t.wfrag = w->w_tail_frag; t.b1 = w->b_ff1;
  t.b2 = w->b_ff2; t.xb = d_xb; t.ssq_out = d_ssq_out;
  LAUNCH(launch_layer_tail(t, (hipStream_t)stream), "layer tail");
  return BT_OK;
}

int bt_gemm3(void* stream, const bt_gemm3_args* a) {
  if (!a || !a->A || !a->W) return bt_set_error(BT_ERR_ARG, "null argument");
  Gemm3P g;
  memset(&g, 0, sizeof g);
  g.A = a->A; g.lda = a->lda; g.M = a->M; g.K = a->K; g.W = a->W; g.N = a->N; g.epi = a->epi; g.bias = a->bias;
  g.ssq_in = a->ssq_in; g.ssq_parts = a->ssq_parts; g.out = a->out; g.ldo = a->ldo; g.x = a->x; g.ldx = a->ldx;
  g.xb = a->xb; g.ssq_out = a->ssq_out; g.n_seq = a->n_seq; g.L = a->L; g.nblk = (a->L + 31) / 32; g.nbp = a->nbp;
  g.heads = a->heads; g.inner = a->heads * 32; g.rope = a->rope; g.qf = a->qf; g.kf = a->kf; g.vf = a->vf;
  g.gates = a->gates; g.b_gates = a->b_gates;
  g.x3 = a->x3; g.status = a->status;
  g.no_resid = a->no_resid; g.gelu = a->gelu; g.conv_C2 = a->conv_C2; g.conv_T = a->conv_T; g.conv_F = a->conv_F;
  if (!gemm3_supported(g)) return bt_set_error(BT_ERR_ARG, "shape not supported by bt_gemm3");
  LAUNCH(launch_gemm3(g, (hipStream_t)stream), "gemm3");
  return BT_OK;
}

int bt_gemm_mx8(void* stream, const void* d_A, const void* d_SA, const void* d_W, const void* d_SW, float* d_out, int M, int N, int K,
                int64_t ldo) {
  GemmMx8P g;
  g.A = d_A; g.SA = d_SA; g.W = d_W; g.SW = d_SW; g.out = d_out; g.ldo = (long)ldo; g.M = M; g.N = N; g.K = K;
  if (!d_A || !d_SA || !d_W || !d_SW || !d_out || !gemm_mx8_supported(g)) return bt_set_error(BT_ERR_ARG, "bad argument to bt_gemm_mx8");
  LAUNCH(launch_gemm_mx8(g, (hipStream_t)stream), "MX e4m3 gemm");
  return BT_OK;
}

int bt_attn_frag_blocks(int L) { return L > 0 ? attn_frag_blocks(L) : 0; }

int bt_attention_frag(void* stream, const bt_attn_frag_args* a) {
  if (!a || !a->q || !a->k || !a->v || !a->gates || !a->out) return bt_set_error(BT_ERR_ARG, "null argument");
  AttnFragP p;
  memset(&p, 0, sizeof p);
  p.q = a->q; p.k = a->k; p.v = a->v; p.gates = a->gates; p.out = a->out; p.n_seq = a->n_seq; p.L = a->L;
  p.heads = a->heads; p.inner = a->inner; p.nbp = a->nbp; p.o_div = a->o_div; p.o_outer = a->o_outer;
  p.o_inner = a->o_inner; p.o_tok = a->o_tok;
  p.x3 = a->x3; p.out_f32 = a->out_f32; p.status = a->status; p.fix_mask = a->scratch;
  if (p.x3 > 0 && !p.fix_mask) return bt_set_error(BT_ERR_ARG, "bt_attention_frag: x3 needs the scratch words (overflow map)");
  LAUNCH(launch_attn_frag(p, (hipStream_t)stream), "attention (fragment-major)");
  return BT_OK;
}

int bt_qkv_front(void* stream, int prec, const bt_pair_weights* w, const float* d_rope, const float* d_x, int B, int T, int F,
                 void* d_q, void* d_k, void* d_v, float* d_gates, int nbp) {
  if (prec != BT_PREC_HALF && prec != BT_PREC_F32X3) return bt_set_error(BT_ERR_ARG, "bt_qkv_front: BT_PREC_HALF or BT_PREC_F32X3");
  const bool x3 = prec == BT_PREC_F32X3;
  const void* wf = !w ? nullptr : x3 ? w->w_qkv_frag_x3 : w->w_qkv_frag;
  if (!w || !wf || !d_rope || !d_x || !d_q || !d_k || !d_v || !d_gates || w->dim > 128)
    return bt_set_error(BT_ERR_ARG, "bad argument to bt_qkv_front");
  QkvFrontP p;
  memset(&p, 0, sizeof p);
  p.x = d_x; p.B = B; p.T = T; p.F = F; p.C = w->dim; p.wfrag = wf; p.b_gates = w->b_gates; p.rope = d_rope;
  p.q = d_q; p.k = d_k; p.v = d_v; p.gates = d_gates; p.nbp = nbp; p.x3 = x3;
  LAUNCH(launch_qkv_front(p, (hipStream_t)stream), "frontend qkv projection");
  return BT_OK;
}

}
```

beat_this_amd/csrc/frontend.hip:

```cpp
#include "common.h"
#include "kernels.h"

namespace {

constexpr int STEM_TT = 8;
__global__ __launch_bounds__(256) void stem_kernel(const StemP p, int t_tiles) {
  __shared__ __attribute__((aligned(16))) float in[STEM_TT + 2][128];
  const int tid = threadIdx.x;
  const int b = blockIdx.x / t_tiles, t0 = (blockIdx.x - b * t_tiles) * STEM_TT;
  for (int i = tid; i < (STEM_TT + 2) * 128; i += 256) {
    const int row = i >> 7, mel = i & 127;
    const int tt = t0 + row - 1;
    float v = 0.f;
    if (tt >= 0 && tt < p.T) v = fmaf(p.spect[((long)b * p.T + tt) * 128 + mel], p.bn1_scale[mel], p.bn1_shift[mel]);
    in[row][mel] = v;
  }
  const int c4 = tid & 7, f = tid >> 3;
  float w[4][12], bias[4];
#pragma unroll
  for (int j = 0; j < 4; ++j) {
#pragma unroll
    for (int i = 0; i < 12; ++i) w[j][i] = p.w[(4 * c4 + j) * 12 + i];
    bias[j] = p.bias[4 * c4 + j];
  }
  __syncthreads();
#pragma unroll
  for (int tt = 0; tt < STEM_TT; ++tt) {
    if (t0 + tt >= p.T) break;
    float a[4] = {bias[0], bias[1], bias[2], bias[3]};
#pragma unroll
    for (int dt = 0; dt < 3; ++dt) {
      const f32x4 v = *reinterpret_cast<const f32x4*>(&in[tt + dt][4 * f]);
#pragma unroll
      for (int df = 0; df < 4; ++df)
#pragma unroll
        for (int j = 0; j < 4; ++j) a[j] = fmaf(w[j][df * 3 + dt], v[df], a[j]);
    }
    *reinterpret_cast<f32x4*>(p.x + ((long)b * p.T + t0 + tt) * 1024 + f * 32 + 4 * c4) =
        f32x4{gelu_erf(a[0]), gelu_erf(a[1]), gelu_erf(a[2]), gelu_erf(a[3])};
  }
}

__global__ __launch_bounds__(256) void head_kernel(const HeadP p) {
  const int lane = threadIdx.x & 63;
  const long row = (long)blockIdx.x * 4 + (threadIdx.x >> 6);
  if (row >= p.M) return;
  const float* x = p.x + row * p.D;
  float ss = 0.f, d0 = 0.f, d1 = 0.f;
  if ((p.D & 3) == 0) {
    for (int k = 4 * lane; k < p.D; k += 256) {
      const f32x4 v = *reinterpret_cast<const f32x4*>(x + k);
      const f32x4 w0 = *reinterpret_cast<const f32x4*>(p.w + k), w1 = *reinterpret_cast<const f32x4*>(p.w + p.D + k);
#pragma unroll
      for (int i = 0; i < 4; ++i) {
        ss = fmaf(v[i], v[i], ss);
        d0 = fmaf(v[i], w0[i], d0);
        d1 = fmaf(v[i], w1[i], d1);
      }
    }
  } else {
    for (int k = lane; k < p.D; k += 64) {
      float v = x[k];
      ss = fmaf(v, v, ss);
      d0 = fmaf(v, p.w[k], d0);
      d1 = fmaf(v, p.w[p.D + k], d1);
    }
  }
#pragma unroll
  for (int o = 32; o > 0; o >>= 1) {
    ss += __shfl_xor(ss, o);
    d0 += __shfl_xor(d0, o);
    d1 += __shfl_xor(d1, o);
  }
  if (lane == 0) {
    const float sc = p.prenorm ? 1.f : sqrtf((float)p.D) / fmaxf(sqrtf(ss), 1e-12f);
    const float y0 = d0 * sc + p.b0, y1 = d1 * sc + p.b1;
    p.beat[row] = p.sum_head ? y0 + y1 : y0;
    p.downbeat[row] = y1;
    if (p.status && !(fabsf(y0) <= 3.0e38f && fabsf(y1) <= 3.0e38f)) atomicOr(p.status, 2);
  }
}

__global__ __launch_bounds__(256) void norm_out_kernel(const float* __restrict__ x, const float* __restrict__ gamma,
                                                       float* __restrict__ y, long M, int D, int* __restrict__ status) {
  const int lane = threadIdx.x & 63;
  const long row = (long)blockIdx.x * 4 + (threadIdx.x >> 6);
  if (row >= M) return;
  const float* xr = x + row * D;
  float ss = 0.f;
  for (int k = lane; k < D; k += 64) ss = fmaf(xr[k], xr[k], ss);
#pragma unroll
  for (int o = 32; o > 0; o >>= 1) ss += __shfl_xor(ss, o);
  const float sc = sqrtf((float)D) / fmaxf(sqrtf(ss), 1e-12f);
  for (int k = lane; k < D; k += 64) y[row * D + k] = xr[k] * sc * gamma[k];
  if (status && lane == 0 && !(ss <= 3.0e38f)) atomicOr(status, 2);
}

__global__ __launch_bounds__(256) void finite_rows_kernel(const float* __restrict__ x, long M, int D, int* __restrict__ status) {
  const int lane = threadIdx.x & 63;
  const long row = (long)blockIdx.x * 4 + (threadIdx.x >> 6);
  if (row >= M) return;
  float ss = 0.f;
  for (int k = lane; k < D; k += 64) ss = fmaf(x[row * D + k], x[row * D + k], ss);
#pragma unroll
  for (int o = 32; o > 0; o >>= 1) ss += __shfl_xor(ss, o);
  if (lane == 0 && !(ss <= 3.0e38f)) atomicOr(status, 2);
}

__global__ __launch_bounds__(256) void shadow_ssq_kernel(const float* __restrict__ x, hf* __restrict__ xb,
                                                         float* __restrict__ ssq, long M, int D, int hl32) {
  const int lane = threadIdx.x & 63;
  const long row = (long)blockIdx.x * 4 + (threadIdx.x >> 6);
  if (row >= M) return;
  for (int g = 0; g < D / 64; ++g) {
    const float v = x[row * D + g * 64 + lane];
    if (hl32) {
      const hf h = (hf)v;
      hf* d = xb + (row * D + g * 64) * 2 + (lane >> 5) * 64 + (lane & 31);
      d[0] = h;
      d[32] = (hf)(v - (float)h);
    } else {
      xb[row * D + g * 64 + lane] = (hf)v;
    }
    float sq = v * v;
#pragma unroll
    for (int o = 32; o > 0; o >>= 1) sq += __shfl_xor(sq, o);
    if (ssq && lane == 0) ssq[(long)g * M + row] = sq;
  }
}

__device__ __forceinline__ long piece_chunk_start(int b, int B, long n, int T, int border) {
  return (b == B - 1 && n > T - 2 * border) ? n - (T - border) : (long)b * (T - 2 * border) - border;
}

__global__ void split_kernel(const float* __restrict__ spect, const int* __restrict__ table, const int* __restrict__ starts,
                             long n_frames, int B, int T, float* __restrict__ chunks, int border) {
  const long total = (long)B * T * 32;
  for (long i = (long)blockIdx.x * blockDim.x + threadIdx.x; i < total; i += (long)gridDim.x * blockDim.x) {
    long row = i >> 5;
    int c4 = (int)(i & 31);
    int b = (int)(row / T), t = (int)(row - (long)b * T);
    long src, lo = 0, hi = n_frames;
    if (table) { src = (long)table[4 * b] + t; lo = table[4 * b + 1]; hi = table[4 * b + 2]; }
    else if (starts) src = (long)starts[b] + t;
    else src = piece_chunk_start(b, B, n_frames, T, border) + t;
    f32x4 v = f32x4{0.f, 0.f, 0.f, 0.f};
    if (src >= lo && src < hi) v = reinterpret_cast<const f32x4*>(spect + src * 128)[c4];
    reinterpret_cast<f32x4*>(chunks + row * 128)[c4] = v;
  }
}

__global__ void aggregate_kernel(const float* __restrict__ cb, const float* __restrict__ cd,
                                 const int* __restrict__ starts, const int* __restrict__ table,
                                 const int* __restrict__ pieces, int B, int T, int border, long n_frames,
                                 float* __restrict__ beat, float* __restrict__ downbeat) {
  long f_lo = 0, f_hi = n_frames;
  int c_lo = 0, c_hi = B;
  if (pieces) {
    const int* pc = pieces + 4 * blockIdx.y;
    f_lo = pc[0]; f_hi = pc[1]; c_lo = pc[2]; c_hi = pc[3];
  }
  for (long i = f_lo + (long)blockIdx.x * blockDim.x + threadIdx.x; i < f_hi; i += (long)gridDim.x * blockDim.x) {
    float vb = -1000.0f, vd = -1000.0f;
    for (int c = c_lo; c < c_hi; ++c) {
      long s = table ? table[4 * c] : starts ? starts[c] : piece_chunk_start(c, B, n_frames, T, border);
      if (i >= s + border && i < s + T - border) {
        vb = cb[(long)c * T + (i - s)];
        vd = cd[(long)c * T + (i - s)];
        break;
      }
    }
    beat[i] = vb;
    downbeat[i] = vd;
  }
}

__global__ __launch_bounds__(1024) void peaks_kernel(const float* __restrict__ logits, long n_uniform,
                                                     const int* __restrict__ spans, int* __restrict__ idx,
                                                     int* __restrict__ count) {
  __shared__ int wave_tot[16];
  __shared__ int base_s;
  const long off = spans ? (long)spans[2 * blockIdx.x] : (long)blockIdx.x * n_uniform;
  const long n = spans ? (long)spans[2 * blockIdx.x + 1] : n_uniform;
  const float* x = logits + off;
  int* out = idx + off;
// ... 128 lines not shown
      const float hq[8] = {ha[0], ha[1], ha[2], ha[3], hb[0], hb[1], hb[2], hb[3]};
#pragma unroll
      for (int e = 0; e < 8; ++e)
#pragma unroll
        for (int j = 0; j < DEC_R; ++j) acc[j] = fmaf(hq[e], w[8 + j - e], acc[j]);
      hi0 = lo0; hi1 = lo1;
    }
  }
  const long m0 = mb + 8L * tid;
  float* yo = y + tr.out_off + m0;
  if (m0 + 8 <= n_out && ((reinterpret_cast<uintptr_t>(yo) & 15) == 0)) {
    *reinterpret_cast<f32x4*>(yo) = f32x4{acc[0], acc[1], acc[2], acc[3]};
    *reinterpret_cast<f32x4*>(yo + 4) = f32x4{acc[4], acc[5], acc[6], acc[7]};
  } else {
#pragma unroll
    for (int j = 0; j < DEC_R; ++j)
      if (m0 + j < n_out) yo[j] = acc[j];
  }
}

}

int launch_resample(const bt_span_t& one, const bt_span_t* tracks, int n_tracks, long max_n_out, int up, int down,
                    const float* h, int half, float* y, hipStream_t s) {
  const int ntaps = 2 * half + 1;
  if (up == 1 && (down == 2 || down == 3 || down == 4)) {
    const int QP = ((ntaps + down - 1) / down + 7) & ~7;
    const size_t smem = (size_t)down * (DEC_OUT + QP) * 4 + (size_t)down * QP * 4;
    if (smem <= 64 * 1024) {
      dim3 grid((unsigned)((max_n_out + DEC_OUT - 1) / DEC_OUT), (unsigned)n_tracks);
      if (down == 2) hipLaunchKernelGGL(decimate_kernel<2>, grid, dim3(256), smem, s, one, tracks, h, half, y);
      else if (down == 3) hipLaunchKernelGGL(decimate_kernel<3>, grid, dim3(256), smem, s, one, tracks, h, half, y);
      else hipLaunchKernelGGL(decimate_kernel<4>, grid, dim3(256), smem, s, one, tracks, h, half, y);
      return (int)hipGetLastError();
    }
  }
  hipLaunchKernelGGL(resample_kernel, dim3((unsigned)((max_n_out + 255) / 256), (unsigned)n_tracks), dim3(256), 0, s, one,
                     tracks, up, down, h, half, y);
  return (int)hipGetLastError();
}

int launch_stem(const StemP& p, hipStream_t s) {
  const int t_tiles = (p.T + STEM_TT - 1) / STEM_TT;
  hipLaunchKernelGGL(stem_kernel, dim3((unsigned)((long)p.B * t_tiles)), dim3(256), 0, s, p, t_tiles);
  return (int)hipGetLastError();
}
__global__ void clear_words_kernel(int* __restrict__ w, int n) {
  if ((int)threadIdx.x < n) w[threadIdx.x] = 0;
}
int launch_clear_words(int* w, int n, hipStream_t s) {
  hipLaunchKernelGGL(clear_words_kernel, dim3(1), dim3(64), 0, s, w, n);
  return (int)hipGetLastError();
}
int launch_head(const HeadP& p, hipStream_t s) {
  hipLaunchKernelGGL(head_kernel, dim3((unsigned)((p.M + 3) / 4)), dim3(256), 0, s, p);
  return (int)hipGetLastError();
}
int launch_norm_out(const float* x, const float* gamma, float* y, long M, int D, hipStream_t s, int* status) {
  hipLaunchKernelGGL(norm_out_kernel, dim3((unsigned)((M + 3) / 4)), dim3(256), 0, s, x, gamma, y, M, D, status);
  return (int)hipGetLastError();
}
int launch_finite_rows(const float* x, long M, int D, int* status, hipStream_t s) {
  hipLaunchKernelGGL(finite_rows_kernel, dim3((unsigned)((M + 3) / 4)), dim3(256), 0, s, x, M, D, status);
  return (int)hipGetLastError();
}
int launch_shadow_ssq(const float* x, void* xb, float* ssq, long M, int D, hipStream_t s, int hl32) {
  if (D % 64 != 0) return -2;
  hipLaunchKernelGGL(shadow_ssq_kernel, dim3((unsigned)((M + 3) / 4)), dim3(256), 0, s, x, reinterpret_cast<hf*>(xb), ssq, M, D, hl32);
  return (int)hipGetLastError();
}
int launch_split(const float* spect, long n_frames, const int* starts, const int* table, int B, int T, float* chunks,
                 hipStream_t s, int border) {
  long total = (long)B * T * 32;
  unsigned grid = (unsigned)((total + 255) / 256 < 8192 ? (total + 255) / 256 : 8192);
  hipLaunchKernelGGL(split_kernel, dim3(grid), dim3(256), 0, s, spect, table, starts, n_frames, B, T, chunks, border);
  return (int)hipGetLastError();
}
int launch_aggregate(const float* cb, const float* cd, const int* starts, const int* table, const int* pieces, int n_pieces,
                     int B, int T, int border, long n_frames, float* beat, float* downbeat, hipStream_t s) {
  unsigned grid = (unsigned)((n_frames + 255) / 256 < 2048 ? (n_frames + 255) / 256 : 2048);
  hipLaunchKernelGGL(aggregate_kernel, dim3(grid, (unsigned)(pieces ? n_pieces : 1)), dim3(256), 0, s, cb, cd, starts, table,
                     pieces, B, T, border, n_frames, beat, downbeat);
  return (int)hipGetLastError();
}
int launch_peaks(const float* logits, long n, const int* spans, int n_arrays, int* idx, int* count, hipStream_t s) {
  hipLaunchKernelGGL(peaks_kernel, dim3((unsigned)n_arrays), dim3(1024), 0, s, logits, n, spans, idx, count);
  return (int)hipGetLastError();
}
```

beat_this_amd/csrc/gemm3.hip:

```cpp
#include <cstdlib>

#include "common.h"
#include "kernels.h"

struct G3CfgS { static constexpr int BM = 128, BN = 128, BK = 32, WGM = 2, WGN = 2, NST = 3, OCC = 3; };
struct G3CfgB { static constexpr int BM = 256, BN = 256, BK = 64, WGM = 2, WGN = 4, NST = 2, OCC = 1; };
struct G3CfgT { static constexpr int BM = 192, BN = 256, BK = 64, WGM = 2, WGN = 4, NST = 2, OCC = 1; };
struct G3CfgSX { static constexpr int BM = 128, BN = 128, BK = 64, WGM = 2, WGN = 2, NST = 2, OCC = 2; };
struct G3CfgBX { static constexpr int BM = 256, BN = 256, BK = 64, WGM = 2, WGN = 4, NST = 2, OCC = 1; };
struct G3CfgTX { static constexpr int BM = 192, BN = 256, BK = 64, WGM = 2, WGN = 4, NST = 2, OCC = 1; };
struct G3CfgMX { static constexpr int BM = 256, BN = 128, BK = 32, WGM = 2, WGN = 2, NST = 3, OCC = 2; };
struct G3CfgHX { static constexpr int BM = 64, BN = 128, BK = 64, WGM = 2, WGN = 2, NST = 3, OCC = 2; };

#ifndef X3_NSPLIT
#define X3_NSPLIT 2
#endif

namespace {

typedef G3CfgS CfgS;
typedef G3CfgB CfgB;

constexpr unsigned OOB = 0x80000000u;

// ... 166 lines not shown
  for (int r = 0; r < 16; ++r) {
    const int h = n0 - 3 * p.inner + crow(r, g);
    if (h < p.heads) p.gates[((long)tseq * p.heads + h) * p.nbp * 32 + t] = sigmoidf(fmaf(acc[r], rs, p.b_gates[h]));
  }
}

template <int EPI, typename CFG, int X3 = 0, int ABL = 0>
__global__ __launch_bounds__(64 * CFG::WGM * CFG::WGN, (CFG::OCC * CFG::WGM * CFG::WGN + 3) / 4)
void gemm3_kernel(const Gemm3P p, int n_tiles, int total_tiles, int per_xcd, int nsplit) {
  constexpr int BM = CFG::BM, BN = CFG::BN, BK = CFG::BK, NST = CFG::NST;
  constexpr int NW = CFG::WGM * CFG::WGN, NT = 64 * NW;
  constexpr int TB = BM / CFG::WGM / 32;
  constexpr int FB = BN / CFG::WGN / 32;
  constexpr int ROWB = BK * 2;
  constexpr int KR = X3 ? BK / 2 : BK;
  constexpr bool HL16 = X3 && BK == 32;
  constexpr int EB = X3 ? 4 : 2;
  constexpr int CPR = ROWB / 16;
  constexpr int RPI = 64 / CPR;
  constexpr int A_BYTES = BM * ROWB, W_BYTES = BN * ROWB, ST_BYTES = A_BYTES + W_BYTES;
  constexpr int APC = A_BYTES / (NT * 16), WPC = W_BYTES / (NT * 16);
  static_assert(EPI != G3_QKV || TB == FB, "the V columns swap the operand roles: square wave tile needed");
  static_assert(BN / CFG::WGN == 64, "ssq partials are per 64 columns = one wave");
  static_assert(!X3 || ROWB == 128 || ROWB == 64, "hl32: a k-step is a whole group (128 B per row) or half of one (64 B)");
  static_assert(X3 != 2 || ROWB == 128, "hl8: a k-step is a whole 32-column group");
  static_assert(NST * ST_BYTES >= NW * 8192, "the epilogues stage 8 KB per wave in the ring's LDS");
  __shared__ __attribute__((aligned(16))) char smem[NST * ST_BYTES];
  const int bid = blockIdx.x;
  int m_tile, n_tile;
  if (nsplit <= 1) {
    const int tile = (bid & 7) * per_xcd + (bid >> 3);
    if (tile >= total_tiles) return;
    m_tile = tile / n_tiles;
    n_tile = tile - m_tile * n_tiles;
  } else {
    const int xcd = bid & 7, slot = bid >> 3;
    const int g = xcd % nsplit, j = xcd / nsplit, per_m = 8 / nsplit, nt = n_tiles / nsplit;
    const int m_local = slot / nt;
    m_tile = m_local * per_m + j;
    n_tile = g * nt + (slot - m_local * nt);
    if ((long)m_tile * n_tiles >= total_tiles) return;
  }
  const int m0 = m_tile * BM, n0 = n_tile * BN;
  const int tid = threadIdx.x, lane = tid & 63, wave = __builtin_amdgcn_readfirstlane(tid >> 6);
  const int g = lane >> 5, lr = lane & 31;
  const int wm = wave / CFG::WGN, wn = wave % CFG::WGN;
  const int nk = p.K / KR;
  auto swz = [](int r) { return ROWB == 64 ? (r >> 2) & 3 : (r >> 1) & 7; };
  const int Lv = p.nblk * 32;

  int kind = 0;
  if constexpr (EPI == G3_QKV) kind = n0 < 3 * p.inner ? n0 / p.inner : 3;
  const bool normal = EPI == G3_QKV && kind == 2;
  if constexpr (BT_QKV_GATE_TILE && EPI == G3_QKV && X3 == 1 && ABL == 0 && BM == 128 && BN == 128 && ROWB == 128 && NW == 4) {
    if (kind == 3 && p.heads <= 32 && (p.x3 & 15) != 3) {
      qkv_gate_tile_x3<CFG>(p, smem, m0, n0, n_tiles, lane, wave);
      return;
    }
  }

  const unsigned a_bytes = (unsigned)((long)p.M * p.lda * EB), w_bytes = (unsigned)((long)n_tiles * BN * p.K * EB);
  static_assert(APC >= 1 && WPC >= 1, "tile too small for the workgroup");
  static_assert(APC <= 4 && WPC <= 4, "voffA / voffW hold at most 4 pieces");
  unsigned voffA[4], voffW[4];
  int tapmask[4] = {0, 0, 0, 0};
#pragma unroll
  for (int i = 0; i < APC; ++i) {
    const int r = (i * NW + wave) * RPI + lane / CPR;
    const int c = (lane % CPR) ^ swz(r);
    long row = (long)m0 + r;
    bool ok = row < p.M;
    if constexpr (EPI == G3_QKV) {
      const int seq = (int)(row / Lv), t = (int)(row - (long)seq * Lv);
      ok = seq < p.n_seq && t < p.L;
      row = (long)seq * p.L + t;
    }
#ifdef BT_ABL_HID_WRAP
    if (EPI == G3_RESID && X3 && p.K >= 1024 && p.conv_C2 == 0) row &= BT_ABL_HID_WRAP - 1;
#endif
    voffA[i] = ok ? (unsigned)(row * p.lda * EB + (HL16 ? (c >> 1) * 64 + (c & 1) * 16 : c * 16)) : OOB;
    if constexpr (EPI == G3_RESID) {
      const int t = p.conv_C2 > 0 ? (int)((row / p.conv_F) % p.conv_T) : 1;
      tapmask[i] = ok ? ((t >= 1 ? 1 : 0) | 2 | (t + 1 < p.conv_T ? 4 : 0)) : 0;
    }
  }
#pragma unroll
  for (int i = 0; i < WPC; ++i) {
    const int r = (i * NW + wave) * RPI + lane / CPR;
    const int c = (lane % CPR) ^ swz(r);
    voffW[i] = (unsigned)((long)(n0 + r) * p.K * EB + (HL16 ? (c >> 1) * 64 + (c & 1) * 16 : c * 16));
  }
  const bool conv = EPI == G3_RESID && p.conv_C2 > 0;
  const unsigned tap_bytes = conv ? (unsigned)(p.conv_F * p.conv_C2 * EB) : 0u;
  const int c2_shift = conv ? __builtin_ctz((unsigned)p.conv_C2) : 0;
  const rsrc_t rA = __builtin_amdgcn_make_buffer_rsrc(const_cast<char*>(reinterpret_cast<const char*>(p.A)) - tap_bytes, 0,
                                                      a_bytes + 2 * tap_bytes, 0x00020000);
  const rsrc_t rW = __builtin_amdgcn_make_buffer_rsrc(const_cast<void*>(p.W), 0, w_bytes, 0x00020000);
#define G3_ISSUE(kt, stage)                                                                                          \
  do {                                                                                                                \
    char* st_ = smem + (stage) * ST_BYTES + wave * 1024;                                                              \
    const int so_ = HL16 ? ((kt) >> 1) * 128 + ((kt) & 1) * 32 : (kt) * ROWB;                                         \
    if (conv) {                                                                                                       \
      const int tap_ = ((kt) * KR) >> c2_shift;                                                                       \
      const int kin_ = ((kt) * KR) & (p.conv_C2 - 1);                                                                 \
      const int soa_ = tap_ * (int)tap_bytes + (HL16 ? (kin_ >> 5) * 128 + ((kin_ >> 4) & 1) * 32 : kin_ * EB);      \
      _Pragma("unroll") for (int i_ = 0; i_ < APC; ++i_)                                                              \
// ... 562 lines not shown
```

beat_this_amd/csrc/kernels.h:

```cpp
#pragma once
#include <hip/hip_runtime.h>
#include <stdint.h>

#ifndef BT_PREC_F32
#define BT_PREC_F32 0
#define BT_PREC_HALF 1
#endif
#ifndef BT_PREC_F32X3
#define BT_PREC_F32X3 3
#endif

enum {
  GEMM_EPI_STORE = 0,
  GEMM_EPI_RESID = 1,
  GEMM_EPI_QKV = 2
};
enum {
  GEMM_F_RMS = 1,
  GEMM_F_BIAS = 2,
  GEMM_F_GELU = 4,
  GEMM_F_OUT_F32 = 8,
  GEMM_F_A_F32 = 16,
  GEMM_F_CONV = 32,
  GEMM_F_ROWMAP = 64
};

struct GemmP {
  const void* A;
  long lda;
  const void* W;
  int M, N, K;
  int epi, flags;
  const float* bias;
  void* out;
  long ldo;
  float* x;
  long ldx;
  void* xb;
  float* ssq_out;
  int conv_C2, conv_T, conv_F;
  float* gates;
  int inner;
  int heads;
  const float* rope;
  int pdiv, pmod;
  int map_T, map_F;
};
int launch_gemm(const GemmP& p, int prec, hipStream_t s);

enum { G3_FF1 = 0, G3_RESID = 1, G3_QKV = 2 };
struct Gemm3P {
  const void* A; long lda; int M, K;
  const void* W; int N;
  int epi;
  const float* bias;
  const float* ssq_in; int ssq_parts;
  void* out; long ldo;
  float* x; long ldx; void* xb;
  float* ssq_out;
  int n_seq, L, nblk, nbp, heads, inner;
  const float* rope; void* qf; void* kf; void* vf; float* gates; const float* b_gates;
  int no_resid;
  int gelu;
  int conv_C2, conv_T, conv_F;
  int x3;
  int* status;
};
enum { G3_X3_F8 = 0x100, G3_X3_OUT_F8 = 0x200 };
bool gemm3_supported(const Gemm3P& p);
int launch_gemm3(const Gemm3P& p, hipStream_t s);

struct GemmMx8P {
  const void* A; const void* SA;
  const void* W; const void* SW;
  float* out; long ldo;
  int M, N, K;
};
bool gemm_mx8_supported(const GemmMx8P& p);
int launch_gemm_mx8(const GemmMx8P& p, hipStream_t s);

struct AttnP {
  const void* qkv;
  long ld;
  const float* gates;
  void* out;
  int n_seq, L, heads, inner;
  int o_div;
  long o_outer, o_inner, o_tok;
};
int launch_attn_flash(const AttnP& p, int prec, hipStream_t s);

struct AttnFragP {
  const void* q; const void* k; const void* v;
  const float* gates;
  void* out;
  int n_seq, L, heads, inner, nbp;
  int o_div;
  long o_outer, o_inner, o_tok;
  int x3, out_f32;
  int* status;
  int* fix_mask;
};
int attn_frag_blocks(int L);
int launch_attn_frag(const AttnFragP& p, hipStream_t s);

struct QkvFrontP {
  const float* x;
  int B, T, F, C;
  const void* wfrag;
  const float* b_gates;
  const float* rope;
  void* q; void* k; void* v;
  float* gates;
  int nbp;
  int x3;
  int* status;
};
int launch_qkv_front(const QkvFrontP& p, hipStream_t s);

struct FusedFFP {
  float* x; long M; int C;
  const void* wfrag;
  const float* b1; const float* b2;
  void* xb;
};
int launch_ff_fused(const FusedFFP& p, int prec, hipStream_t s);

struct FusedOutFFP {
  float* x; long M; int C;
  const void* ao;
  const void* wfrag;
  const float* b1; const float* b2;
  void* xb;
  int abl;
  int shadow_only;
};
int launch_outff_fused(const FusedOutFFP& p, int prec, hipStream_t s);
struct FusedAttnFFP {
  float* x; long M; int C;
  const float* b_gates; const float* rope;
  const void* wfrag;
  const float* b1; const float* b2;
};
int launch_attnff_fused(const FusedAttnFFP& p, int prec, hipStream_t s);

struct LayerTailP {
  float* x; long M; int C; int hidden;
  const void* ao;
  const void* wfrag;
  const float* b1; const float* b2;
  void* xb;
  float* ssq_out;
};
bool layer_tail_supported(int C, int hidden);
int launch_layer_tail(const LayerTailP& p, hipStream_t s);

struct StemP {
  const float* spect;
  float* x;
  const float* bn1_scale; const float* bn1_shift;
  const float* w;
  const float* bias;
  int B, T;
};
int launch_stem(const StemP& p, hipStream_t s);

struct HeadP {
  const float* x;
  const float* w;
  float b0, b1;
  float* beat; float* downbeat;
  int M, D, sum_head;
  int prenorm;
  int* status;
};
int launch_head(const HeadP& p, hipStream_t s);
int launch_clear_words(int* w, int n, hipStream_t s);
int launch_norm_out(const float* x, const float* gamma, float* y, long M, int D, hipStream_t s, int* status = nullptr);
int launch_finite_rows(const float* x, long M, int D, int* status, hipStream_t s);
int launch_shadow_ssq(const float* x, void* xb, float* ssq, long M, int D, hipStream_t s, int hl32 = 0);

struct bt_span_t { const float* data; long n; long out_off; long n_out; };

int launch_split(const float* spect, long n_frames, const int* starts, const int* table, int B, int T, float* chunks,
                 hipStream_t s, int border = 0);
int launch_aggregate(const float* cb, const float* cd, const int* starts, const int* table, const int* pieces, int n_pieces,
                     int B, int T, int border, long n_frames, float* beat, float* downbeat, hipStream_t s);
int launch_resample(const bt_span_t& one, const bt_span_t* tracks, int n_tracks, long max_n_out, int up, int down,
                    const float* h, int half, float* y, hipStream_t s);
int launch_peaks(const float* logits, long n, const int* spans, int n_arrays, int* idx, int* count, hipStream_t s);

struct LogmelP {
  bt_span_t one;
  const bt_span_t* tracks;
  int n_tracks; long max_frames;
  const float* window;
  const float* twiddle;
  const int* mel_start;
  const int* mel_len;
  const float* mel_w;
  float* spect;
};
int launch_logmel(const LogmelP& p, hipStream_t s);
```

beat_this_amd/inference.py:

```python
from __future__ import annotations

import inspect

import numpy as np
import torch

from . import _lib
from .model import BeatThis
from .pack import Engine
from .postprocessor import PendingBeats, Postprocessor, _host_post
from .preprocessing import LogMelSpect, load_audio
from .utils import replace_state_dict_key, save_beat_tsv

CHECKPOINT_URL = "https://cloud.cp.jku.at/public.php/dav/files/7ik4RrBKTS273gp"
MAX_CHUNKS_PER_LAUNCH = 96
CONCURRENT_STREAMS = 2
CONCURRENT_SLICE_CHUNKS = 32
_SIDE_STREAMS: dict = {}


def _side_streams(main, n):
    key = (main, n)
    if key not in _SIDE_STREAMS:
        _SIDE_STREAMS[key] = [torch.cuda.Stream(main.device) for _ in range(n)]
# ... 405 lines not shown
                                    for k in range(len(frame_off) - 1)])
        pending.logits = (beat, down, frame_off)
        if checks:
            return _GuardedPending(pending, self.model.engine(), checks,
                                   lambda: self._frames2beats_async(spect, frame_off, _lib.PREC_F32))
        return pending


class _GuardedPending:

    def __init__(self, inner, eng, checks, redo):
        self.inner, self.eng, self.checks, self.redo = inner, eng, checks, redo
        self.logits = inner.logits

    def result(self):
        out = self.inner.result()
        if self.checks and self.eng.range_exceeded(self.checks):
            self.inner = self.redo()
            self.logits = self.inner.logits
            out = self.inner.result()
        self.checks = self.redo = None
        return out


class File2Beats(Audio2Beats):
    def __call__(self, audio_path):
        signal, sr = load_audio(audio_path)
        return super().__call__(signal, sr)


class File2File(File2Beats):
    def __call__(self, audio_path, output_path):
        downbeats, beats = super().__call__(audio_path)
        save_beat_tsv(downbeats, beats, output_path)


_RESAMPLE_FILTERS: dict = {}


def _resample_filter(up: int, down: int, device):
    from . import tables

    key = (up, down, torch.device(device))
    if key not in _RESAMPLE_FILTERS:
        h, half = tables.resample_filter(up, down)
        _RESAMPLE_FILTERS[key] = (torch.from_numpy(h.astype(np.float32)).to(device), half)
    return _RESAMPLE_FILTERS[key]


def batch_predict_aggregate(spect: torch.Tensor, frame_off, chunk_size: int, border_size: int, model, checks=None):
    return _batch_predict(spect, frame_off, chunk_size, border_size, model, _model_precision(model), checks)


def _batch_predict(spect, frame_off, chunk_size, border_size, model, prec, checks):
    if prec != _lib.PREC_F32X3:
        checks = None
    elif checks is None:
        flags = []
        out = _batch_predict(spect, frame_off, chunk_size, border_size, model, prec, flags)
        if not model.engine().range_exceeded(flags):
            return out
        prec = _lib.PREC_F32
    _lib.require_gpu(spect, "spectrogram")
    if spect.dim() != 2 or spect.shape[1] != 128:
        raise ValueError(f"expected a (frames, 128) spectrogram, got {tuple(spect.shape)}")
    spect = spect.to(torch.float32).contiguous()
    dev = spect.device
    frame_off = np.asarray(frame_off, dtype=np.int64)
    total = int(frame_off[-1])
    both = torch.empty((2, total), dtype=torch.float32, device=dev)
    beat, down = both[0], both[1]
    rows, pieces = [], []
    for k in range(len(frame_off) - 1):
        lo, hi = int(frame_off[k]), int(frame_off[k + 1])
        n = hi - lo
        if n == 0:
            continue
        if n <= chunk_size - 2 * border_size:
            r = _split_predict(spect[lo:hi], chunk_size, border_size, "keep_first", model, prec, checks)
            beat[lo:hi], down[lo:hi] = r["beat"], r["downbeat"]
            continue
        c0 = len(rows)
        rows += [(lo + int(st), lo, hi, 0) for st in chunk_starts(n, chunk_size, border_size)]
        pieces.append((lo, hi, c0, len(rows)))
    if not rows:
        return beat, down
    if total + chunk_size >= 2 ** 31:
        raise ValueError("batch too long for 32-bit frame indices: split the track list")
    B = len(rows)
    tab = _lib.upload(np.concatenate([np.asarray(rows, dtype=np.int32).reshape(-1), np.asarray(pieces, dtype=np.int32).reshape(-1)]), dev)
    d_rows, d_pieces = tab[: 4 * B], tab[4 * B:]
    cb = torch.empty((B, chunk_size), dtype=torch.float32, device=dev)
    cd = torch.empty((B, chunk_size), dtype=torch.float32, device=dev)
    lib, st = _lib.lib(), _lib.stream_ptr(dev)
    n_slices = -(-B // MAX_CHUNKS_PER_LAUNCH)
    if B >= CONCURRENT_SLICE_CHUNKS and CONCURRENT_STREAMS > 1:
        n_slices = max(n_slices, CONCURRENT_STREAMS)
    step = -(-B // n_slices)
    with torch.cuda.device(dev):
        main = torch.cuda.current_stream(dev)
        side = _side_streams(main, min(n_slices, CONCURRENT_STREAMS)) if n_slices > 1 and CONCURRENT_STREAMS > 1 else [main]
        if side[0] is not main:
            ready = torch.cuda.Event()
            ready.record(main)
        for j, i in enumerate(range(0, B, step)):
            nb = min(step, B - i)
            st_ = side[j % len(side)]
            with torch.cuda.stream(st_):
                if st_ is not main:
                    st_.wait_event(ready)
                chunks = torch.empty((nb, chunk_size, 128), dtype=torch.float32, device=dev)
                _lib.check(lib.bt_split_chunks_batch(_lib.stream_ptr(dev), spect.data_ptr(), d_rows[4 * i:].data_ptr(), nb,
                                                     chunk_size, chunks.data_ptr()))
                if isinstance(model, BeatThis) and not _model_hooked(model):
                    model._run(chunks, 0, 2, out=(cb[i: i + nb], cd[i: i + nb]), prec=prec, checks=checks)
                else:
                    r = model(chunks)
                    cb[i: i + nb], cd[i: i + nb] = r["beat"], r["downbeat"]
        for st_ in side:
            if st_ is not main:
                main.wait_stream(st_)
        st = _lib.stream_ptr(dev)
        max_frames = max(hi - lo for lo, hi, _, _ in pieces)
        _lib.check(lib.bt_aggregate_batch(st, cb.data_ptr(), cd.data_ptr(), d_rows.data_ptr(), d_pieces.data_ptr(),
                                          len(pieces), max_frames, chunk_size, border_size, beat.data_ptr(),
                                          down.data_ptr()))
    return beat, down


def resample_gpu(signal: torch.Tensor, in_rate: int, out_rate: int) -> torch.Tensor:
    from math import gcd

    _lib.require_gpu(signal, "waveform")
    if signal.dim() != 1:
        raise ValueError(f"expected a 1-D waveform, got shape {tuple(signal.shape)}")
    in_rate, out_rate = int(in_rate), int(out_rate)
    g = gcd(in_rate, out_rate)
    up, down = out_rate // g, in_rate // g
    if up == down:
        return signal
    h, half = _resample_filter(up, down, signal.device)
    x = signal.to(torch.float32).contiguous()
    n_in = x.shape[0]
    n_out = -(-n_in * up // down)
    y = torch.empty(n_out, dtype=torch.float32, device=x.device)
    with torch.cuda.device(x.device):
        _lib.check(_lib.lib().bt_resample(_lib.stream_ptr(x.device), x.data_ptr(), n_in, up, down, h.data_ptr(), half,
                                          y.data_ptr(), n_out))
    return y
```

beat_this_amd/model/__init__.py:

```python
from __future__ import annotations

import weakref

import torch
from torch import nn

from .. import _lib
from . import backward as _bw
from ..pack import Engine, PackedModel
from ..weights import random_state_dict, resolve_hparams, state_dict_shapes

_BUFFER_LEAVES = ("running_mean", "running_var", "num_batches_tracked")
_TREE_EPOCH = [0]


class _TracksChildren:

    def __setattr__(self, name, value):
        if isinstance(value, (nn.Module, nn.Parameter)):
            _TREE_EPOCH[0] += 1
        super().__setattr__(name, value)

    def __delattr__(self, name):
        _TREE_EPOCH[0] += 1
# ... 269 lines not shown

    def _unit_train(self, x: torch.Tensor, kind: str, node: nn.Module) -> torch.Tensor:
        D = self.hparams["transformer_dim"]
        _lib.require_gpu(x, "sub-module input")
        if self.device.type != "cuda":
            self.engine()
        if x.dim() != 3 or x.shape[2] != D:
            raise ValueError(f"expected a (batch, time, {D}) input, got {tuple(x.shape)}")
        if x.shape[0] == 0 or x.shape[1] == 0:
            return _bw.empty_with_graph(x.shape, x, _params_of(node))
        x = x.to(torch.float32)
        mixed = self.train_precision == "16-mixed"
        if kind == "attn":
            return _bw.attention(node, x, *self._rope(x.shape[1]), self._next_dropout(), mixed)
        return _bw.feedforward(node, x, self._next_dropout(), mixed) if kind == "ff" else _bw.final_norm(node, x)

    def _head_train(self, x: torch.Tensor) -> dict:
        D = self.hparams["transformer_dim"]
        _lib.require_gpu(x, "stage input")
        if self.device.type != "cuda":
            self.engine()
        if x.dim() != 3 or x.shape[2] != D:
            raise ValueError(f"expected a (batch, time, {D}) input, got {tuple(x.shape)}")
        if x.shape[0] == 0 or x.shape[1] == 0:
            params = _params_of(self.task_heads)
            return {"beat": _bw.empty_with_graph(x.shape[:2], x, params), "downbeat": _bw.empty_with_graph(x.shape[:2], x, params)}
        beat, down = _bw.head(self.task_heads, x.to(torch.float32), self.hparams["sum_head"])
        return {"beat": beat, "downbeat": down}

    def forward(self, x: torch.Tensor) -> dict:
        if x.dim() != 3:
            raise ValueError(f"expected (batch, time, {self.hparams['spect_dim']}) input, got {tuple(x.shape)}")
        _lib.require_gpu(x, "model input")
        if torch.is_grad_enabled():
            self._refuse_trainable_frontend()
            if self._differentiable(None, self.transformer_blocks) or self._differentiable(None, self.task_heads):
                with torch.no_grad():
                    h = self.frontend(x)
                return self.task_heads(self.transformer_blocks(h))
        if x.shape[0] == 0 or x.shape[1] == 0:
            empty = torch.empty((x.shape[0], x.shape[1]), dtype=torch.float32, device=x.device)
            return {"beat": empty, "downbeat": empty.clone()}
        if _hooked_below(self):
            return self.task_heads(self.transformer_blocks(self.frontend(x)))
        beat, down = self._run(x, 0, 2)
        return {"beat": beat, "downbeat": down}

    def _precision(self) -> int:
        half = torch.is_autocast_enabled("cuda") if hasattr(torch, "is_autocast_enabled") else False
        if half:
            return _lib.PREC_HALF
        return _lib.PREC_F32X3 if self.fp32_split_gemms and not _lib.lib().bt_half_is_bf16() else _lib.PREC_F32

    def _run(self, x: torch.Tensor, first: int, last: int, out=None, prec=None, checks=None):
        if x.dim() != 3:
            raise ValueError(f"expected a (batch, time, features) input, got {tuple(x.shape)}")
        _lib.require_gpu(x, "stage input")
        if x.shape[0] == 0 or x.shape[1] == 0:
            D = self.hparams["transformer_dim"]
            empty = torch.empty((x.shape[0], x.shape[1]), dtype=torch.float32, device=x.device)
            return (empty, empty.clone()) if last == 2 else torch.empty((x.shape[0], x.shape[1], D), dtype=torch.float32, device=x.device)
        prec = self._precision() if prec is None else prec
        return self.engine(frontend_only=last == 0).forward_stages(x, prec, first, last, logits_out=out, checks=checks)

    def _run_unit(self, x: torch.Tensor, kind: str, index: int):
        _lib.require_gpu(x, "sub-module input")
        if kind in ("attn", "ff", "norm"):
            tb = self.transformer_blocks
            node = tb.norm if kind == "norm" else tb.layers[index][0 if kind == "attn" else 1]
            if self._differentiable(x, node):
                return self._unit_train(x, kind, node)
        half = torch.is_autocast_enabled("cuda") if hasattr(torch, "is_autocast_enabled") else False
        prec = _lib.PREC_HALF if half else _lib.PREC_F32
        eng = self.engine()
        D = self.hparams["transformer_dim"]

        def to_btfc(t, i):
            c, f = 32 << i, 32 >> i
            if t.dim() != 4 or t.shape[1] != c or t.shape[2] != f:
                raise ValueError(f"expected a (batch, {c}, {f}, time) input, got {tuple(t.shape)}")
            return t.permute(0, 3, 2, 1).contiguous()

        def partial(t, i):
            if not self.hparams["partial_transformers"]:
                return t
            return eng.forward_unit(t, prec, _lib.UNIT_PARTIAL, i, t.shape)

        def conv(t, i):
            b, n, f, c = t.shape
            return eng.forward_unit(t, prec, _lib.UNIT_CONV, i, (b, n, f // 2, 2 * c))

        if kind == "stem":
            if x.dim() != 3 or x.shape[2] != 128:
                raise ValueError(f"expected a (batch, time, 128) input, got {tuple(x.shape)}")
            return eng.forward_unit(x, prec, _lib.UNIT_STEM, 0, (x.shape[0], x.shape[1], 32, 32)).permute(0, 3, 2, 1)
        if kind == "partial":
            return partial(to_btfc(x, index), index).permute(0, 3, 2, 1)
        if kind == "block":
            blk = self.frontend.blocks[index]
            if _hooked_below(blk) and "partial" in blk._modules:
                return conv(to_btfc(blk.partial(x), index), index).permute(0, 3, 2, 1)
            return conv(partial(to_btfc(x, index), index), index).permute(0, 3, 2, 1)
        if kind == "blocks":
            if _hooked_below(self.frontend.blocks):
                for blk in self.frontend.blocks:
                    x = blk(x)
                return x
            t = to_btfc(x, 0)
            for i in range(3):
                t = conv(partial(t, i), i)
            return t.permute(0, 3, 2, 1)
        if kind == "concat":
            if x.dim() != 4:
                raise ValueError(f"expected a (batch, channels, freq, time) input, got {tuple(x.shape)}")
            b, c, f, n = x.shape
            return x.permute(0, 3, 1, 2).reshape(b, n, c * f)
# ... 21 lines not shown
```

beat_this_amd/pack.py:

```python
from __future__ import annotations

import collections
import ctypes as C
import math
import threading

import torch

from . import _lib, tables

LOG2E = 1.4426950408889634
BN_EPS = 1e-5


def perm32(w: torch.Tensor) -> torch.Tensor:
    idx = torch.tensor([(r & 3) + 8 * (r >> 2) + 4 * g for g in range(2) for r in range(16)])
    n, k = w.shape
    return w.reshape(n, k // 32, 32)[:, :, idx].reshape(n, k).contiguous()


def fragment_tiles(w: torch.Tensor) -> torch.Tensor:
    r, k = w.shape
    t = w.reshape(r // 32, 32, k // 32, 2, 16)
    return t.permute(0, 2, 3, 1, 4).reshape(r // 32, k // 32, 64, 16)
# ... 324 lines not shown
    def _rebuild_handle(self, undo) -> None:
        torch.cuda.synchronize(self.device)
        lib, h = _lib.lib(), C.c_void_p()
        try:
            _lib.check(lib.bt_engine_create(C.byref(self.packed.desc), C.byref(h)))
            for name, opt in self.OPTIONS.items():
                _lib.check(lib.bt_engine_set_option(h, opt, self.get_option(name)))
        except Exception:
            if h.value:
                lib.bt_engine_destroy(h)
            undo()
            raise
        old, self._h = self._h, h
        lib.bt_engine_destroy(old)
        self._drop_graphs()

    def get_option(self, name: str) -> int:
        v = C.c_int(0)
        _lib.check(_lib.lib().bt_engine_get_option(self._h, self.OPTIONS[name], C.byref(v)))
        return int(v.value)

    def ensure_positions(self, T: int) -> None:
        if T <= self.packed.desc.rope_len:
            return
        p = self.packed
        old = p.desc.rope, p.desc.rope_len, p._rope_t
        p.set_positions(-(-T // 512) * 512)

        def undo():
            p.desc.rope, p.desc.rope_len, p._rope_t = old
        self._rebuild_handle(undo)

    def _workspace(self, need: int) -> torch.Tensor:
        key = torch.cuda.current_stream(self.device)
        ws, small = self._ws.pop(key, (None, 0))
        if ws is not None and ws.numel() < need:
            ws = None
        elif ws is not None and ws.numel() > 4 * need:
            small += 1
            if small >= self.SHRINK_AFTER:
                ws = None
        else:
            small = 0
        if ws is None:
            ws, small = torch.empty(need, dtype=torch.uint8, device=self.device), 0
        self._ws[key] = (ws, small)
        while len(self._ws) > self.MAX_WORKSPACES:
            self._ws.popitem(last=False)
        return ws

    def forward(self, spect: torch.Tensor, prec: int):
        return self.forward_stages(spect, prec, 0, 2)

    def forward_stages(self, spect: torch.Tensor, prec: int, first: int, last: int, logits_out=None, checks=None):
        _lib.require_gpu(spect, "stage input")
        B, T, M = spect.shape
        D = self.packed.desc.transformer_dim
        if M != (128 if first == 0 else D):
            raise ValueError(f"expected {128 if first == 0 else D} input features, got {M}")
        x = spect.to(torch.float32).contiguous()
        self.ensure_positions(T)
        need = _lib.lib().bt_workspace_bytes(self._h, B, T, prec)
        if need == 0:
            raise ValueError("empty batch")
        ws = self._workspace(need)
        beat = down = out = None
        if last == 2 and logits_out is not None:
            beat, down = logits_out
            for t in (beat, down):
                if t.dtype != torch.float32 or tuple(t.shape) != (B, T) or not t.is_contiguous() or t.device != x.device:
                    raise ValueError("logits_out: two contiguous fp32 (batch, time) tensors on the input's device")
        elif last == 2:
            beat = torch.empty((B, T), dtype=torch.float32, device=self.device)
            down = torch.empty((B, T), dtype=torch.float32, device=self.device)
        else:
            out = torch.empty((B, T, D), dtype=torch.float32, device=self.device)
        with torch.cuda.device(self.device):
            _lib.check(_lib.lib().bt_forward_stages(self._h, _lib.stream_ptr(self.device), prec, first, last, x.data_ptr(), B, T,
                                                    ws.data_ptr(), ws.numel(), _lib.ptr(out), _lib.ptr(beat), _lib.ptr(down)))
            if prec == _lib.PREC_F32X3:
                flag = ws[:4].view(torch.int32)
                if checks is not None:
                    host = torch.empty(1, dtype=torch.int32, pin_memory=True)
                    host.copy_(flag, non_blocking=True)
                    ev = torch.cuda.Event()
                    ev.record(torch.cuda.current_stream(self.device))
                    checks.append((host, ev))
                elif int(flag.item()) != 0:
                    self._count_fallback()
                    return self.forward_stages(spect, _lib.PREC_F32, first, last, logits_out=logits_out)
        return (beat, down) if last == 2 else out

    def forward_unit(self, x: torch.Tensor, prec: int, unit: int, index: int, out_shape) -> torch.Tensor:
        _lib.require_gpu(x, "sub-module input")
        B, T = int(x.shape[0]), int(x.shape[1])
        if B == 0 or T == 0:
            raise ValueError("empty batch")
        if prec == _lib.PREC_F32X3:
            prec = _lib.PREC_F32
        x = x.to(torch.float32).contiguous()
        self.ensure_positions(T)
        ws = self._workspace(_lib.lib().bt_workspace_bytes(self._h, B, T, prec))
        out = torch.empty(tuple(out_shape), dtype=torch.float32, device=self.device)
        with torch.cuda.device(self.device):
            _lib.check(_lib.lib().bt_forward_unit(self._h, _lib.stream_ptr(self.device), prec, unit, index, x.data_ptr(),
                                                  out.data_ptr(), B, T, ws.data_ptr(), ws.numel()))
        return out

    GRAPH_MAX_CHUNKS = 11
    GRAPH_T = 1500
    GRAPH_MAX_ENTRIES = 12

    def graph_forward(self, B: int, T: int, prec: int):
        if not self._graphs_ok or T != self.GRAPH_T or B > self.GRAPH_MAX_CHUNKS or self.profiling:
            return None
        stream = torch.cuda.current_stream(self.device)
        key = (stream, B, T, prec)
        e = self._graphs.pop(key, None)
        if e is None:
            try:
                e = _GraphEntry(self, B, T, prec, stream)
            except Exception as err:
                self._graphs_ok = False
                self._graph_error = repr(err)
                return None
        cache = self._graphs
        cache[key] = e
        while len(cache) > self.GRAPH_MAX_ENTRIES:
            cache.popitem(last=False)
        return e

    def _graph_workspace(self, stream, need: int) -> torch.Tensor:
        pool = self._graph_ws
        ws = pool.get(stream)
        if ws is None or ws.numel() < need:
            ws = pool[stream] = torch.empty(need, dtype=torch.uint8, device=self.device)
        return ws

    def _a2b_workspace(self, need: int) -> torch.Tensor:
        stream = torch.cuda.current_stream(self.device)
        pool = self._a2b_ws
        ws, small = pool.get(stream, (None, 0))
        if ws is not None and ws.numel() > 4 * need:
# ... 62 lines not shown
```

include/beat_this_amd.h:

```cpp
#ifndef BEAT_THIS_AMD_H
#define BEAT_THIS_AMD_H
#include <stddef.h>
#include <stdint.h>

#ifdef __cplusplus
extern "C" {
#endif

#define BT_OK 0
#define BT_ERR_ARG (-1)
#define BT_ERR_HIP (-2)
#define BT_ERR_WORKSPACE (-3)

#define BT_PREC_F32 0
#define BT_PREC_HALF 1

#define BT_PREC_F32X3 3

#define BT_MAX_LAYERS 32

typedef struct bt_engine bt_engine;

typedef struct {
  int32_t dim, heads;
// ... 22 lines not shown
  const void* w_ff2_f8;
} bt_pair_weights;

typedef struct {
  int32_t transformer_dim, n_layers, sum_head, partial_transformers;
  const float* bn1_scale;
  const float* bn1_shift;
  const float* stem_w;
  const float* stem_b;
  bt_pair_weights front[3][2];
  const void* conv_w[3][2];
  const float* conv_b[3];
  const void* lin_w[2];
  const float* lin_b;
  bt_pair_weights layers[BT_MAX_LAYERS];
  const float* head_w;
  float head_b[2];
  const float* rope;
  int32_t ff_mult;
  const float* norm_out_g;
  const float* head_w_raw;
  const void* conv_w_x3[3];
  const void* lin_w_x3;
  int32_t rope_len;
} bt_model_desc;

typedef struct {
  const float* window;
  const float* twiddle;
  const int32_t* mel_start;
  const int32_t* mel_len;
  const float* mel_w;
} bt_logmel_tables;

const char* bt_last_error(void);
#define BT_ABI_VERSION 600
int bt_version(void);
int bt_half_is_bf16(void);
void bt_struct_sizes(int32_t* out);

int bt_engine_create(const bt_model_desc* desc, bt_engine** out);
void bt_engine_destroy(bt_engine* e);
#define BT_OPT_X3_ATTN_P16 1
#define BT_OPT_X3_GEMM_FP8 2
#define BT_OPT_WS_GUARD 3
int bt_engine_set_option(bt_engine* e, int option, int value);
int bt_engine_get_option(const bt_engine* e, int option, int* value);
size_t bt_workspace_bytes(const bt_engine* e, int B, int T, int prec);
int bt_workspace_regions(const bt_engine* e, int B, int T, int prec, int64_t* begin_end, int max);

int bt_forward(bt_engine* e, void* stream, int prec, const float* d_spect, int B, int T, void* d_ws,
               size_t ws_bytes, float* d_beat, float* d_downbeat);

int bt_forward_stages(bt_engine* e, void* stream, int prec, int first, int last, const float* d_in, int B, int T, void* d_ws,
                      size_t ws_bytes, float* d_out, float* d_beat, float* d_downbeat);

enum { BT_UNIT_STEM = 0, BT_UNIT_PARTIAL = 1, BT_UNIT_CONV = 2, BT_UNIT_LINEAR = 3, BT_UNIT_ATTN = 4, BT_UNIT_FF = 5, BT_UNIT_NORM = 6,
       BT_UNIT_FRONT_ATTN = 7, BT_UNIT_FRONT_FF = 8 };
int bt_forward_unit(bt_engine* e, void* stream, int prec, int unit, int index, const float* d_in, float* d_out, int B, int T,
                    void* d_ws, size_t ws_bytes);

int bt_split_chunks(void* stream, const float* d_spect, int64_t n_frames, const int32_t* d_starts, int B, int T,
                    float* d_chunks);
int bt_aggregate(void* stream, const float* d_chunk_beat, const float* d_chunk_downbeat, const int32_t* d_starts,
                 int B, int T, int border, int64_t n_frames, float* d_beat, float* d_downbeat);

int bt_logmel(void* stream, const bt_logmel_tables* tables, const float* d_audio, int64_t n_samples,
              float* d_spect);

typedef struct { const float* d_in; int64_t n_in; int64_t out_off; int64_t n_out; } bt_span;
int bt_resample_batch(void* stream, const bt_span* d_tracks, int n_tracks, int64_t max_n_out, int up, int down,
                      const float* d_filter, int half_len, float* d_out);
int bt_logmel_batch(void* stream, const bt_logmel_tables* tables, const bt_span* d_tracks, int n_tracks,
                    int64_t max_frames, float* d_spect);
int bt_split_chunks_batch(void* stream, const float* d_spect, const int32_t* d_chunk_table, int B, int T, float* d_chunks);
int bt_aggregate_batch(void* stream, const float* d_chunk_beat, const float* d_chunk_downbeat, const int32_t* d_chunk_table,
                       const int32_t* d_pieces, int n_pieces, int64_t max_frames, int T, int border, float* d_beat,
                       float* d_downbeat);

int bt_resample(void* stream, const float* d_in, int64_t n_in, int up, int down, const float* d_filter, int half_len,
                float* d_out, int64_t n_out);

int bt_peaks(void* stream, const float* d_logits, int64_t n, int n_arrays, int32_t* d_idx, int32_t* d_count);
int bt_peaks_batch(void* stream, const float* d_logits, const int32_t* d_spans, int n_arrays, int32_t* d_idx,
                   int32_t* d_count);
int bt_peaks_host(const float* logits, int64_t n, int32_t* idx, int32_t* count);

int bt_dbn_tables(double fps, double min_bpm, double max_bpm, int num_tempi, double transition_lambda,
                  double observation_lambda, double threshold, const int32_t* beats_per_bar, int n_hmm, void* tables,
                  size_t* bytes);
size_t bt_dbn_workspace_bytes(const void* tables, int n_tracks, int64_t total_frames);
int bt_dbn_decode(void* stream, const void* tables, const void* d_tables, const void* d_logits, int f64,
                  const int32_t* d_spans, int n_tracks, int64_t total_frames, int32_t* d_out, void* d_ws, size_t ws_bytes);
int bt_dbn_viterbi(void* stream, const void* tables, const void* d_tables, int hmm, const double* d_dens, int64_t n,
                   int32_t* d_path, double* d_log_prob, void* d_ws, size_t ws_bytes);
int bt_dbn_viterbi_host(const void* tables, int hmm, const double* dens, int64_t n, int32_t* path, double* log_prob);
int bt_dbn_host(const void* tables, const double* beat, const double* downbeat, int64_t n, int32_t* rows, int32_t* n_rows);
int bt_dbn_host_act(const void* tables, const double* act, int64_t n, int32_t* rows, int32_t* n_rows);

#define BT_METRICS_COLS 12
#define BT_METRICS_NONFINITE 1
#define BT_METRICS_UNSORTED 2
#define BT_METRICS_LATE 4
#define BT_METRICS_NEAREST 64
#define BT_METRICS_OFFSETS 128
size_t bt_beat_metrics_workspace_bytes(int n_tracks, int64_t total_ref, int64_t total_est);
// ... 69 lines not shown
                           int use_graph);

#define BT_CAT_STEM 0
#define BT_CAT_QKV_GEMM 1
#define BT_CAT_ATTN_FLASH 2
#define BT_CAT_OUT_GEMM 3
#define BT_CAT_FF1_GEMM 4
#define BT_CAT_FF2_GEMM 5
#define BT_CAT_CONV_GEMM 6
#define BT_CAT_LINEAR_GEMM 7
#define BT_CAT_HEAD 8
#define BT_CAT_FF_FUSED 9
#define BT_CAT_ATTN_FREQ_FUSED 10
#define BT_CAT_LAYER_TAIL 11
#define BT_PROFILE_CATEGORIES 12
void bt_profile_begin(bt_engine* e);
int bt_profile_end(bt_engine* e, double* ms_by_category, int32_t* launches_by_category, int n_categories);

typedef struct {
  const void* A; int64_t lda; const void* W; int32_t M, N, K; int32_t epi, flags;
  const float* bias; void* out; int64_t ldo; float* x; int64_t ldx;
  int32_t conv_C2, conv_T, conv_F;
  float* gates; int32_t inner, heads; const float* rope; int32_t pdiv, pmod, map_T, map_F;
} bt_gemm_args;
int bt_gemm(void* stream, int prec, const bt_gemm_args* a);

typedef struct {
  const void* qkv; int64_t ld; const float* gates; void* out;
  int32_t n_seq, L, heads, inner, o_div; int64_t o_outer, o_inner, o_tok;
} bt_attn_args;
int bt_attention(void* stream, int prec, const bt_attn_args* a);

#define BT_X3_P16 8
typedef struct {
  const void* q; const void* k; const void* v; const float* gates; void* out;
  int32_t n_seq, L, heads, inner, nbp, o_div; int64_t o_outer, o_inner, o_tok;
  int32_t x3, out_f32; int32_t* status;
  int32_t* scratch;
} bt_attn_frag_args;
int bt_gemm_mx8(void* stream, const void* d_A, const void* d_SA, const void* d_W, const void* d_SW, float* d_out, int M, int N,
                int K, int64_t ldo);

typedef struct {
  const void* A; int64_t lda; int32_t M, K; const void* W; int32_t N, epi; const float* bias;
  const float* ssq_in; int32_t ssq_parts; void* out; int64_t ldo; float* x; int64_t ldx; void* xb; float* ssq_out;
  int32_t n_seq, L, nbp, heads; const float* rope; void* qf; void* kf; void* vf; float* gates; const float* b_gates;
  int32_t no_resid;
  int32_t gelu, conv_C2, conv_T, conv_F;
  int32_t x3; int32_t* status;
} bt_gemm3_args;
int bt_gemm3(void* stream, const bt_gemm3_args* a);
int bt_attn_frag_blocks(int L);
int bt_attention_frag(void* stream, const bt_attn_frag_args* a);
int bt_qkv_front(void* stream, int prec, const bt_pair_weights* w, const float* d_rope, const float* d_x, int B, int T, int F,
                 void* d_q, void* d_k, void* d_v, float* d_gates, int nbp);
int bt_ff_fused(void* stream, int prec, const bt_pair_weights* w, float* d_x, int64_t M);
int bt_outff_fused(void* stream, int prec, const bt_pair_weights* w, const void* d_ao, float* d_x, int64_t M, void* d_xb);
int bt_attnff_fused(void* stream, int prec, const bt_pair_weights* w, const float* d_rope, float* d_x, int64_t M);
int bt_layer_tail(void* stream, const bt_pair_weights* w, int hidden, const void* d_ao, float* d_x, int64_t M, void* d_xb,
                  float* d_ssq_out);

#define BT_TRAIN_UNIT_HEAD 16
#define BT_TRAIN_DW_ROWS 1024
#define BT_TRAIN_CS_ROWS 64
#define BT_TRAIN_ATTN_BLOCK 64
typedef struct {
  int32_t B, T, dim, hidden, rope_len, residual, sum_head, reserved;
  const float* rope;
  const float* gamma; const float* w1; const float* b1; const float* w2; const float* b2; const float* w3;
  const float* x; float* y; float* y2; float* save_o; float* save_lse;
  const float* gy; const float* gy2;
  float* gx; float* g_gamma; float* g_w1; float* g_b1; float* g_w2; float* g_b2; float* g_w3;
  void* ws; size_t ws_bytes;
} bt_train_args;
void bt_train_struct_sizes(int32_t* out);
size_t bt_train_workspace_bytes(int unit, int backward, int B, int T, int dim, int hidden);
int bt_train_forward(void* stream, int unit, const bt_train_args* a);
int bt_train_backward(void* stream, int unit, const bt_train_args* a);

#define BT_DROP_ATTN_P 0
#define BT_DROP_ATTN_OUT 1
#define BT_DROP_FF_HIDDEN 2
#define BT_DROP_FF_OUT 3
typedef struct {
  float p; uint32_t reserved; uint64_t seed; uint64_t stream;
} bt_train_dropout;
void bt_train_dropout_struct_sizes(int32_t* out);
size_t bt_train_workspace_bytes_dropout(int unit, int backward, int B, int T, int dim, int hidden);
int bt_train_forward_dropout(void* stream, int unit, const bt_train_args* a, const bt_train_dropout* dropout);
int bt_train_backward_dropout(void* stream, int unit, const bt_train_args* a, const bt_train_dropout* dropout);
void bt_philox4x32_10_host(const uint32_t* ctr, const uint32_t* key, uint32_t* out);
int bt_dropout_mask_host(const bt_train_dropout* dropout, int site, int B, int T, int dim, int hidden, uint8_t* out);

size_t bt_train_workspace_bytes_mixed(int unit, int backward, int B, int T, int dim, int hidden, int with_dropout);
int bt_train_forward_mixed(void* stream, int unit, const bt_train_args* a, const bt_train_dropout* dropout_or_null);
int bt_train_backward_mixed(void* stream, int unit, const bt_train_args* a, const bt_train_dropout* dropout_or_null);
int bt_train_matmul_mixed(void* stream, int form, const float* A, const float* B, int M, int N, int K, float* C);

#define BT_OPTIM_CHUNK 4096
#define BT_OPTIM_NORM_SLICE 4096
#define BT_OPTIM_MAX_GROUPS 8
typedef struct {
  float* param; int64_t offset, numel; int32_t group, reserved;
} bt_optim_tensor;
typedef struct {
  int32_t tensor, chunk;
// ... 25 lines not shown
```

Measured before the change: 63860.

## Skip dead border rows in final transformer layer and head using live ranges

```diff
diff --git a/beat_this_amd/_lib.py b/beat_this_amd/_lib.py
--- a/beat_this_amd/_lib.py
+++ b/beat_this_amd/_lib.py
@@ -168,6 +168,8 @@
     "bt_workspace_regions": (C.c_int, [C.c_void_p, C.c_int, C.c_int, C.c_int, C.POINTER(C.c_int64), C.c_int]),
     "bt_forward": (C.c_int, [C.c_void_p, C.c_void_p, C.c_int, C.c_void_p, C.c_int, C.c_int, C.c_void_p, C.c_size_t,
                              C.c_void_p, C.c_void_p]),
+    "bt_forward_live": (C.c_int, [C.c_void_p, C.c_void_p, C.c_int, C.c_void_p, C.c_int, C.c_int, C.c_void_p, C.c_size_t,
+                                  C.c_void_p, C.c_void_p, C.c_void_p]),
     "bt_forward_stages": (C.c_int, [C.c_void_p, C.c_void_p, C.c_int, C.c_int, C.c_int, C.c_void_p, C.c_int, C.c_int, C.c_void_p,
                                     C.c_size_t, C.c_void_p, C.c_void_p, C.c_void_p]),
     "bt_forward_unit": (C.c_int, [C.c_void_p, C.c_void_p, C.c_int, C.c_int, C.c_int, C.c_void_p, C.c_void_p, C.c_int, C.c_int,
@@ -198,6 +200,8 @@
     "bt_gemm": (C.c_int, [C.c_void_p, C.c_int, C.POINTER(GemmArgs)]),
     "bt_attention": (C.c_int, [C.c_void_p, C.c_int, C.POINTER(AttnArgs)]),
     "bt_gemm3": (C.c_int, [C.c_void_p, C.POINTER(Gemm3Args)]),
+    "bt_gemm3_live": (C.c_int, [C.c_void_p, C.POINTER(Gemm3Args), C.c_void_p, C.c_int]),
+    "bt_attention_frag_live": (C.c_int, [C.c_void_p, C.POINTER(AttnFragArgs), C.c_void_p]),
     "bt_gemm_mx8": (C.c_int, [C.c_void_p, C.c_void_p, C.c_void_p, C.c_void_p, C.c_void_p, C.c_void_p, C.c_int, C.c_int, C.c_int, C.c_int64]),
     "bt_attn_frag_blocks": (C.c_int, [C.c_int]),
     "bt_attention_frag": (C.c_int, [C.c_void_p, C.POINTER(AttnFragArgs)]),
diff --git a/beat_this_amd/csrc/attn2.hip b/beat_this_amd/csrc/attn2.hip
--- a/beat_this_amd/csrc/attn2.hip
+++ b/beat_this_amd/csrc/attn2.hip
@@ -981,6 +981,20 @@
   }
 }
 
+DEVI bool attn_dead_wg(const AttnFragP& p, int sh, int qb, int n, int nblk) {
+  const int seq = sh / p.heads;
+  const int lo = max(p.live[2 * seq], qb * 32), hi = min(p.live[2 * seq + 1], min((qb + n) * 32, p.L));
+  if (lo < hi) return false;
+  const int j = threadIdx.x;
+  if (j < n && qb + j < nblk) p.fix_mask[(long)sh * p.nbp + qb + j] = 0;
+  return true;
+}
+DEVI bool attn_live_blk(const AttnFragP& p, int sh, int blk) {
+  if (!p.live) return true;
+  const int seq = sh / p.heads;
+  return max(p.live[2 * seq], blk * 32) < min(p.live[2 * seq + 1], blk * 32 + 32);
+}
+
 template <int QB, int OUT, int KBX, int MINW, bool P16>
 __global__ __launch_bounds__(256, MINW) void attn_frag_x3_kernel(const AttnFragP p, int nqt, int sh_total) {
   constexpr int TILEX_BYTES = KBX * BLKX_BYTES;
@@ -990,6 +1004,7 @@
   const int sh = (idx / nqt) * 8 + (bid & 7);
   const int qt = idx % nqt;
   if (sh >= sh_total) return;
+  if (p.live && attn_dead_wg(p, sh, qt * 4 * QB, 4 * QB, (p.L + 31) >> 5)) return;
   const int tid = threadIdx.x, lane = tid & 63, wave = __builtin_amdgcn_readfirstlane(tid >> 6);
   const int g = lane >> 5, lr = lane & 31;
   const int L = p.L;
@@ -1027,7 +1042,7 @@
     const bool valid = qb0 + j < nblk && (qb0 + j) * 32 + lr < L;
     bad[j] = valid && !(l_tot[j] < 65504.f);
     const unsigned long long bw = __ballot(bad[j]);
-    if (lane == 0 && qb0 + j < nblk) p.fix_mask[(long)sh * p.nbp + qb0 + j] = (int)(unsigned)bw;
+    if (lane == 0 && qb0 + j < nblk) p.fix_mask[(long)sh * p.nbp + qb0 + j] = attn_live_blk(p, sh, qb0 + j) ? (int)(unsigned)bw : 0;
   }
 #ifdef BT_DEV
   if (p.status && tid == 0) atomicAdd(p.status + 2, 1);
@@ -1056,6 +1071,7 @@
   const int sh = (idx / nqt) * 8 + (bid & 7);
   const int qt = idx % nqt;
   if (sh >= sh_total) return;
+  if (p.live && attn_dead_wg(p, sh, qt * 4 * QB, 4 * QB, (p.L + 31) >> 5)) return;
   const int tid = threadIdx.x, lane = tid & 63, wave = __builtin_amdgcn_readfirstlane(tid >> 6);
   const int g = lane >> 5, lr = lane & 31;
   const int L = p.L;
@@ -1215,7 +1231,7 @@
     const bool valid = qb0 + j < nblk && (qb0 + j) * 32 + lrE < L;
     bad[j] = valid && !(l_tot[j] < 65504.f);
     const unsigned long long bw = __ballot(bad[j]);
-    if (laneE == 0 && qb0 + j < nblk) p.fix_mask[(long)sh * p.nbp + qb0 + j] = (int)(unsigned)bw;
+    if (laneE == 0 && qb0 + j < nblk) p.fix_mask[(long)sh * p.nbp + qb0 + j] = attn_live_blk(p, sh, qb0 + j) ? (int)(unsigned)bw : 0;
   }
 #ifdef BT_DEV
   if (p.status && tid == 0) atomicAdd(p.status + 2, 1);
diff --git a/beat_this_amd/csrc/common.h b/beat_this_amd/csrc/common.h
--- a/beat_this_amd/csrc/common.h
+++ b/beat_this_amd/csrc/common.h
@@ -66,6 +66,18 @@
 }
 
 DEVI int crow(int r, int g) { return (r & 3) + 8 * (r >> 2) + 4 * g; }
+
+DEVI bool rows_all_dead(const int* __restrict__ live, int len, int n, long r0, long r1) {
+  r1 = r1 < (long)n * len ? r1 : (long)n * len;
+  if (r0 >= r1) return false;
+  const int c0 = (int)(r0 / len), c1 = (int)((r1 - 1) / len);
+  for (int c = c0; c <= c1; ++c) {
+    const long base = (long)c * len;
+    const long a = base + live[2 * c], b = base + live[2 * c + 1];
+    if ((a > r0 ? a : r0) < (b < r1 ? b : r1)) return false;
+  }
+  return true;
+}
 
 DEVI float gelu_erf(float x) {
   const float t = __builtin_amdgcn_rcpf(fmaf(0.2316418882f, fabsf(x), 1.0f));
diff --git a/beat_this_amd/csrc/engine.hip b/beat_this_amd/csrc/engine.hip
--- a/beat_this_amd/csrc/engine.hip
+++ b/beat_this_amd/csrc/engine.hip
@@ -165,7 +165,7 @@
   HeadP p;
   p.x = x; p.w = w; p.b0 = d.head_b[0]; p.b1 = d.head_b[1];
   p.beat = beat; p.downbeat = downbeat; p.M = M; p.D = d.transformer_dim; p.sum_head = d.sum_head; p.prenorm = prenorm;
-  p.status = status;
+  p.status = status; p.live = nullptr; p.live_T = 0;
   return p;
 }
 
@@ -188,6 +188,7 @@
   bool next8;
   bool tail;
   bool shadow_dead;
+  const int* live;
 };
 
 enum { LAYERS_GENERIC, LAYERS_FRAG_HALF, LAYERS_FRAG_X3 };
@@ -207,7 +208,10 @@
 #ifndef BT_SKIP_DEAD_STORES
 #define BT_SKIP_DEAD_STORES 1
 #endif
-Route plan_route(const bt_engine& e, int B, int T, int prec, int first, int last, const Workspace& ws) {
+#ifndef BT_LIVE_ROWS
+#define BT_LIVE_ROWS 1
+#endif
+Route plan_route(const bt_engine& e, int B, int T, int prec, int first, int last, const Workspace& ws, const int* d_live = nullptr) {
   const bt_model_desc& d = e.d;
   const int D = d.transformer_dim;
   Route r;
@@ -257,6 +261,7 @@
     f.next8 = frag_x3 && e.x3_gemm_fp8 >= 2 && l + 1 < d.n_layers && d.layers[l + 1].w_qkvg_f8 && w.w_ff2_f8;
     f.tail = frag_half && w.w_tail_frag && layer_tail_supported(D, d.ff_mult * D);
     f.shadow_dead = BT_SKIP_DEAD_STORES && frag_x3 && last == 2 && l == d.n_layers - 1;
+    f.live = BT_LIVE_ROWS && frag_x3 && last == 2 && l == d.n_layers - 1 ? d_live : nullptr;
   }
   return r;
 }
@@ -398,12 +403,13 @@
   g.ssq_in = ws.ssq[0]; g.ssq_parts = parts; g.x3 = r.x3 | (f.qkv8 ? G3_X3_F8 : 0); g.status = status;
   g.n_seq = B; g.L = T; g.nblk = (T + 31) / 32; g.nbp = ws.nbp; g.heads = H; g.inner = D; g.rope = rope;
   g.qf = ws.qf; g.kf = ws.kf; g.vf = ws.vf; g.gates = ws.gates_h; g.b_gates = pw.b_gates;
+  g.live = f.live; g.live_T = T;
   LAUNCH_CAT(CAT_QKV, s, launch_gemm3(g, s), r.x3 ? "qkv gemm (hi + lo)" : "qkv gemm");
   AttnFragP a;
   memset(&a, 0, sizeof a);
   a.q = ws.qf; a.k = ws.kf; a.v = ws.vf; a.gates = ws.gates_h; a.out = ws.ao; a.heads = H; a.inner = D; a.nbp = ws.nbp;
   attn_rows(a, B, T, 1);
-  a.x3 = r.x3_attn; a.out_f32 = f.out8 ? 2 : 0; a.status = status; a.fix_mask = ws.fix_mask;
+  a.x3 = r.x3_attn; a.out_f32 = f.out8 ? 2 : 0; a.status = status; a.fix_mask = ws.fix_mask; a.live = f.live;
   LAUNCH_CAT(CAT_ATTN_FLASH, s, launch_attn_frag(a, s), r.x3 ? "attention (hi + lo)" : "attention");
   if (f.tail) {
     LayerTailP t;
@@ -415,17 +421,18 @@
   memset(&g, 0, sizeof g);
   g.A = ws.ao; g.lda = D; g.M = M; g.K = D; g.W = w(pw.w_out, pw.w_out_x3, pw.w_out_f8, f.out8); g.N = D; g.epi = G3_RESID;
   g.x3 = r.x3 | (f.out8 ? G3_X3_F8 : 0) | (f.ff8 ? G3_X3_OUT_F8 : 0); g.status = status;
-  g.x = ws.xm; g.ldx = D; g.xb = ws.xmb; g.ssq_out = ws.ssq[1];
+  g.x = ws.xm; g.ldx = D; g.xb = ws.xmb; g.ssq_out = ws.ssq[1]; g.live = f.live; g.live_T = T;
   LAUNCH_CAT(CAT_OUT, s, launch_gemm3(g, s), r.x3 ? "out-proj gemm (hi + lo)" : "out-proj gemm");
   memset(&g, 0, sizeof g);
   g.A = ws.xmb; g.lda = D; g.M = M; g.K = D; g.W = w(pw.w_ff1, pw.w_ff1_x3, pw.w_ff1_f8, f.ff8); g.N = HID; g.epi = G3_FF1;
   g.x3 = r.x3 | (f.ff8 ? G3_X3_F8 | G3_X3_OUT_F8 : 0); g.status = status;
-  g.bias = pw.b_ff1; g.ssq_in = ws.ssq[1]; g.ssq_parts = parts; g.out = ws.hid; g.ldo = HID;
+  g.bias = pw.b_ff1; g.ssq_in = ws.ssq[1]; g.ssq_parts = parts; g.out = ws.hid; g.ldo = HID; g.live = f.live; g.live_T = T;
   LAUNCH_CAT(CAT_FF1, s, launch_gemm3(g, s), r.x3 ? "ff1 gemm (hi + lo)" : "ff1 gemm");
   memset(&g, 0, sizeof g);
   g.A = ws.hid; g.lda = HID; g.M = M; g.K = HID; g.W = w(pw.w_ff2, pw.w_ff2_x3, pw.w_ff2_f8, f.ff8); g.N = D; g.epi = G3_RESID;
   g.x3 = r.x3 | (f.ff8 ? G3_X3_F8 : 0) | (f.next8 ? G3_X3_OUT_F8 : 0); g.status = status;
   g.bias = pw.b_ff2; g.x = ws.xm; g.ldx = D; g.xb = f.shadow_dead ? nullptr : ws.xmb; g.ssq_out = f.shadow_dead ? nullptr : ws.ssq[0];
+  g.live = f.live; g.live_T = T;
   LAUNCH_CAT(CAT_FF2, s, launch_gemm3(g, s), r.x3 ? "ff2 gemm (hi + lo)" : "ff2 gemm");
   return BT_OK;
 }
@@ -538,8 +545,21 @@
   return bt_forward_stages(e, stream, prec, 0, 2, d_spect, B, T, d_ws, ws_bytes, nullptr, d_beat, d_downbeat);
 }
 
+static int forward_stages(bt_engine* e, void* stream, int prec, int first, int last, const float* d_spect, int B, int T, void* d_ws,
+                          size_t ws_bytes, float* d_out, float* d_beat, float* d_downbeat, const int* d_live);
+
+int bt_forward_live(bt_engine* e, void* stream, int prec, const float* d_spect, int B, int T, void* d_ws, size_t ws_bytes,
+                    float* d_beat, float* d_downbeat, const int32_t* d_live) {
+  return forward_stages(e, stream, prec, 0, 2, d_spect, B, T, d_ws, ws_bytes, nullptr, d_beat, d_downbeat, d_live);
+}
+
 int bt_forward_stages(bt_engine* e, void* stream, int prec, int first, int last, const float* d_spect, int B, int T, void* d_ws,
                       size_t ws_bytes, float* d_out, float* d_beat, float* d_downbeat) {
+  return forward_stages(e, stream, prec, first, last, d_spect, B, T, d_ws, ws_bytes, d_out, d_beat, d_downbeat, nullptr);
+}
+
+static int forward_stages(bt_engine* e, void* stream, int prec, int first, int last, const float* d_spect, int B, int T, void* d_ws,
+                          size_t ws_bytes, float* d_out, float* d_beat, float* d_downbeat, const int* d_live) {
   if (!e || !d_spect || !d_ws) return bt_set_error(BT_ERR_ARG, "null argument");
   if (first < 0 || last > 2 || first > last) return bt_set_error(BT_ERR_ARG, "stages: need 0 <= first <= last <= 2");
   if (last == 2 ? (!d_beat || !d_downbeat) : !d_out) return bt_set_error(BT_ERR_ARG, "null output");
@@ -554,7 +574,7 @@
   const Workspace ws = carve((char*)d_ws, B, T, D, d.ff_mult, prec, (size_t)e->ws_guard);
   if (ws.total > ws_bytes) return bt_set_error(BT_ERR_WORKSPACE, "workspace too small");
   if (prec == BT_PREC_F32X3 && BT_HALF_IS_BF16) return bt_set_error(BT_ERR_ARG, "BT_PREC_F32X3 needs an IEEE fp16 build");
-  const Route r = plan_route(*e, B, T, prec, first, last, ws);
+  const Route r = plan_route(*e, B, T, prec, first, last, ws, d_live);
   hipStream_t s = (hipStream_t)stream;
   if (r.x3) LAUNCH(launch_clear_words(ws.status, 1, s), "clearing the range flag");
   int* status = r.x3 ? ws.status : nullptr;
@@ -594,7 +614,8 @@
     LAUNCH_CAT(CAT_HEAD, s, launch_norm_out(ws.xm, d.norm_out_g, d_out, (long)B * T, D, s, status), "final norm");
     return BT_OK;
   }
-  const HeadP hp = head_params(d, ws.xm, d.head_w, 0, d_beat, d_downbeat, B * T, status);
+  HeadP hp = head_params(d, ws.xm, d.head_w, 0, d_beat, d_downbeat, B * T, status);
+  if (d.n_layers > 0 && r.layers == LAYERS_FRAG_X3) { hp.live = r.layer[d.n_layers - 1].frag.live; hp.live_T = T; }
   LAUNCH_CAT(CAT_HEAD, s, launch_head(hp, s), "head");
   return BT_OK;
 }
@@ -895,6 +916,13 @@
   lp.tracks = nullptr; lp.n_tracks = 1; lp.max_frames = (long)pl.n_frames;
   LAUNCH(launch_logmel(lp, s), "logmel");
   LAUNCH(launch_split(spect, (long)pl.n_frames, nullptr, nullptr, pl.B, pl.T, chunks, s, border), "split");
+  enum { A2B_LIVE_WORD = 8, A2B_LIVE_MAX = (64 - A2B_LIVE_WORD) / 2 };
+  const int* d_live = nullptr;
+  if (prec == BT_PREC_F32X3 && pl.B <= A2B_LIVE_MAX) {
+    int* tab = (int*)fws + A2B_LIVE_WORD;
+    LAUNCH(launch_live_ranges(tab, pl.B, pl.T, border, (long)pl.n_frames, s), "live row ranges");
+    d_live = tab;
+  }
   const int warm_key = prec << 8 | pl.B;
   const bool graphable = use_graph && pl.T == 1500 && pl.B <= 16 && !e->prof.on &&
                          std::find(e->warm.begin(), e->warm.end(), warm_key) != e->warm.end();
@@ -906,7 +934,7 @@
       hipGraph_t graph = nullptr;
       if (!e->cap_stream && hipStreamCreateWithFlags(&e->cap_stream, hipStreamNonBlocking) != hipSuccess) e->cap_stream = nullptr;
       if (e->cap_stream && hipStreamBeginCapture(e->cap_stream, hipStreamCaptureModeThreadLocal) == hipSuccess) {
-        const int rc = bt_forward_stages(e, e->cap_stream, prec, 0, 2, chunks, pl.B, pl.T, fws, pl.forward_bytes, nullptr, cb, cd);
+        const int rc = forward_stages(e, e->cap_stream, prec, 0, 2, chunks, pl.B, pl.T, fws, pl.forward_bytes, nullptr, cb, cd, d_live);
         const hipError_t he = hipStreamEndCapture(e->cap_stream, &graph);
         hipGraphExec_t exec = nullptr;
         if (rc == BT_OK && he == hipSuccess && graph && hipGraphInstantiate(&exec, graph, nullptr, nullptr, 0) == hipSuccess) {
@@ -929,7 +957,7 @@
     g->stamp = ++e->graph_clock;
     if (hipGraphLaunch(g->exec, s) != hipSuccess) return bt_set_error(BT_ERR_HIP, "replay of the captured forward");
   } else {
-    if (int rc = bt_forward_stages(e, s, prec, 0, 2, chunks, pl.B, pl.T, fws, pl.forward_bytes, nullptr, cb, cd)) return rc;
+    if (int rc = forward_stages(e, s, prec, 0, 2, chunks, pl.B, pl.T, fws, pl.forward_bytes, nullptr, cb, cd, d_live)) return rc;
     if (pl.T == 1500 && pl.B <= 16 && std::find(e->warm.begin(), e->warm.end(), warm_key) == e->warm.end()) e->warm.push_back(warm_key);
   }
   LAUNCH(launch_aggregate(cb, cd, nullptr, nullptr, nullptr, 1, pl.B, pl.T, border, (long)pl.n_frames, beat, downb, s), "aggregate");
@@ -1037,8 +1065,12 @@
   return BT_OK;
 }
 
-int bt_gemm3(void* stream, const bt_gemm3_args* a) {
+int bt_gemm3(void* stream, const bt_gemm3_args* a) { return bt_gemm3_live(stream, a, nullptr, 0); }
+
+int bt_gemm3_live(void* stream, const bt_gemm3_args* a, const int32_t* d_live, int live_T) {
   if (!a || !a->A || !a->W) return bt_set_error(BT_ERR_ARG, "null argument");
+  if (d_live && (a->x3 == 0 || (a->epi == G3_QKV ? live_T != a->L : (live_T <= 0 || a->M % live_T != 0))))
+    return bt_set_error(BT_ERR_ARG, "bt_gemm3_live: x3 launches on whole chunks of live_T rows (QKV: live_T = L)");
   Gemm3P g;
   memset(&g, 0, sizeof g);
   g.A = a->A; g.lda = a->lda; g.M = a->M; g.K = a->K; g.W = a->W; g.N = a->N; g.epi = a->epi; g.bias = a->bias;
@@ -1048,6 +1080,7 @@
   g.gates = a->gates; g.b_gates = a->b_gates;
   g.x3 = a->x3; g.status = a->status;
   g.no_resid = a->no_resid; g.gelu = a->gelu; g.conv_C2 = a->conv_C2; g.conv_T = a->conv_T; g.conv_F = a->conv_F;
+  g.live = d_live; g.live_T = live_T;
   if (!gemm3_supported(g)) return bt_set_error(BT_ERR_ARG, "shape not supported by bt_gemm3");
   LAUNCH(launch_gemm3(g, (hipStream_t)stream), "gemm3");
   return BT_OK;
@@ -1064,7 +1097,9 @@
 
 int bt_attn_frag_blocks(int L) { return L > 0 ? attn_frag_blocks(L) : 0; }
 
-int bt_attention_frag(void* stream, const bt_attn_frag_args* a) {
+int bt_attention_frag(void* stream, const bt_attn_frag_args* a) { return bt_attention_frag_live(stream, a, nullptr); }
+
+int bt_attention_frag_live(void* stream, const bt_attn_frag_args* a, const int32_t* d_live) {
   if (!a || !a->q || !a->k || !a->v || !a->gates || !a->out) return bt_set_error(BT_ERR_ARG, "null argument");
   AttnFragP p;
   memset(&p, 0, sizeof p);
@@ -1073,6 +1108,8 @@
   p.o_inner = a->o_inner; p.o_tok = a->o_tok;
   p.x3 = a->x3; p.out_f32 = a->out_f32; p.status = a->status; p.fix_mask = a->scratch;
   if (p.x3 > 0 && !p.fix_mask) return bt_set_error(BT_ERR_ARG, "bt_attention_frag: x3 needs the scratch words (overflow map)");
+  if (d_live && (p.x3 <= 0 || p.o_div != 1)) return bt_set_error(BT_ERR_ARG, "bt_attention_frag_live: x3 launches with o_div = 1");
+  p.live = d_live;
   LAUNCH(launch_attn_frag(p, (hipStream_t)stream), "attention (fragment-major)");
   return BT_OK;
 }
diff --git a/beat_this_amd/csrc/frontend.hip b/beat_this_amd/csrc/frontend.hip
--- a/beat_this_amd/csrc/frontend.hip
+++ b/beat_this_amd/csrc/frontend.hip
@@ -45,6 +45,10 @@
   const int lane = threadIdx.x & 63;
   const long row = (long)blockIdx.x * 4 + (threadIdx.x >> 6);
   if (row >= p.M) return;
+  if (p.live) {
+    const int c = (int)(row / p.live_T), t = (int)(row - (long)c * p.live_T);
+    if (t < p.live[2 * c] || t >= p.live[2 * c + 1]) return;
+  }
   const float* x = p.x + row * p.D;
   float ss = 0.f, d0 = 0.f, d1 = 0.f;
   if ((p.D & 3) == 0) {
@@ -131,6 +135,19 @@
 
 __device__ __forceinline__ long piece_chunk_start(int b, int B, long n, int T, int border) {
   return (b == B - 1 && n > T - 2 * border) ? n - (T - border) : (long)b * (T - 2 * border) - border;
+}
+
+__global__ void live_ranges_kernel(int* __restrict__ live, int B, int T, int border, long n_frames) {
+  const int b = threadIdx.x;
+  if (b >= B) return;
+  const long s = piece_chunk_start(b, B, n_frames, T, border);
+  long lo = s + border > 0 ? s + border : 0, hi = s + T - border < n_frames ? s + T - border : n_frames;
+  for (int c = 0; c < b; ++c) {
+    const long e = piece_chunk_start(c, B, n_frames, T, border) + T - border;
+    lo = e > lo ? e : lo;
+  }
+  live[2 * b] = hi > lo ? (int)(lo - s) : 0;
+  live[2 * b + 1] = hi > lo ? (int)(hi - s) : 0;
 }
 
 __global__ void split_kernel(const float* __restrict__ spect, const int* __restrict__ table, const int* __restrict__ starts,
@@ -365,6 +382,11 @@
   hipLaunchKernelGGL(clear_words_kernel, dim3(1), dim3(64), 0, s, w, n);
   return (int)hipGetLastError();
 }
+int launch_live_ranges(int* live, int B, int T, int border, long n_frames, hipStream_t s) {
+  if (B <= 0 || B > 64) return -2;
+  hipLaunchKernelGGL(live_ranges_kernel, dim3(1), dim3(64), 0, s, live, B, T, border, n_frames);
+  return (int)hipGetLastError();
+}
 int launch_head(const HeadP& p, hipStream_t s) {
   hipLaunchKernelGGL(head_kernel, dim3((unsigned)((p.M + 3) / 4)), dim3(256), 0, s, p);
   return (int)hipGetLastError();
diff --git a/beat_this_amd/csrc/gemm3.hip b/beat_this_amd/csrc/gemm3.hip
--- a/beat_this_amd/csrc/gemm3.hip
+++ b/beat_this_amd/csrc/gemm3.hip
@@ -242,6 +242,13 @@
   int kind = 0;
   if constexpr (EPI == G3_QKV) kind = n0 < 3 * p.inner ? n0 / p.inner : 3;
   const bool normal = EPI == G3_QKV && kind == 2;
+  if constexpr (X3 != 0 && ABL == 0) {
+    if (p.live && (EPI != G3_QKV || kind == 0 || kind == 3)) {
+      const int len = EPI == G3_QKV ? Lv : p.live_T;
+      const int n = EPI == G3_QKV ? p.n_seq : p.M / p.live_T;
+      if (rows_all_dead(p.live, len, n, m0, (long)m0 + BM)) return;
+    }
+  }
   if constexpr (BT_QKV_GATE_TILE && EPI == G3_QKV && X3 == 1 && ABL == 0 && BM == 128 && BN == 128 && ROWB == 128 && NW == 4) {
     if (kind == 3 && p.heads <= 32 && (p.x3 & 15) != 3) {
       qkv_gate_tile_x3<CFG>(p, smem, m0, n0, n_tiles, lane, wave);
diff --git a/beat_this_amd/csrc/kernels.h b/beat_this_amd/csrc/kernels.h
--- a/beat_this_amd/csrc/kernels.h
+++ b/beat_this_amd/csrc/kernels.h
@@ -65,6 +65,7 @@
   int conv_C2, conv_T, conv_F;
   int x3;
   int* status;
+  const int* live; int live_T;
 };
 enum { G3_X3_F8 = 0x100, G3_X3_OUT_F8 = 0x200 };
 bool gemm3_supported(const Gemm3P& p);
@@ -100,6 +101,7 @@
   int x3, out_f32;
   int* status;
   int* fix_mask;
+  const int* live;
 };
 int attn_frag_blocks(int L);
 int launch_attn_frag(const AttnFragP& p, hipStream_t s);
@@ -173,9 +175,11 @@
   int M, D, sum_head;
   int prenorm;
   int* status;
+  const int* live; int live_T;
 };
 int launch_head(const HeadP& p, hipStream_t s);
 int launch_clear_words(int* w, int n, hipStream_t s);
+int launch_live_ranges(int* live, int B, int T, int border, long n_frames, hipStream_t s);
 int launch_norm_out(const float* x, const float* gamma, float* y, long M, int D, hipStream_t s, int* status = nullptr);
 int launch_finite_rows(const float* x, long M, int D, int* status, hipStream_t s);
 int launch_shadow_ssq(const float* x, void* xb, float* ssq, long M, int D, hipStream_t s, int hl32 = 0);
diff --git a/beat_this_amd/inference.py b/beat_this_amd/inference.py
--- a/beat_this_amd/inference.py
+++ b/beat_this_amd/inference.py
@@ -481,6 +481,20 @@
     return _batch_predict(spect, frame_off, chunk_size, border_size, model, _model_precision(model), checks)
 
 
+def live_row_ranges(rows, pieces, chunk_size: int, border_size: int) -> np.ndarray:
+    starts = np.asarray([r[0] for r in rows], dtype=np.int64)
+    live = np.zeros((len(starts), 2), dtype=np.int32)
+    for f_lo, f_hi, c_lo, c_hi in pieces:
+        reach = int(f_lo)
+        for b in range(int(c_lo), int(c_hi)):
+            s = int(starts[b])
+            lo, hi = max(s + border_size, reach), min(s + chunk_size - border_size, int(f_hi))
+            if hi > lo:
+                live[b] = (lo - s, hi - s)
+            reach = max(reach, s + chunk_size - border_size)
+    return live
+
+
 def _batch_predict(spect, frame_off, chunk_size, border_size, model, prec, checks):
     if prec != _lib.PREC_F32X3:
         checks = None
@@ -517,8 +531,9 @@
     if total + chunk_size >= 2 ** 31:
         raise ValueError("batch too long for 32-bit frame indices: split the track list")
     B = len(rows)
-    tab = _lib.upload(np.concatenate([np.asarray(rows, dtype=np.int32).reshape(-1), np.asarray(pieces, dtype=np.int32).reshape(-1)]), dev)
-    d_rows, d_pieces = tab[: 4 * B], tab[4 * B:]
+    tab = _lib.upload(np.concatenate([np.asarray(rows, dtype=np.int32).reshape(-1), np.asarray(pieces, dtype=np.int32).reshape(-1),
+                                      live_row_ranges(rows, pieces, chunk_size, border_size).reshape(-1)]), dev)
+    d_rows, d_pieces, d_live = tab[: 4 * B], tab[4 * B: 4 * B + 4 * len(pieces)], tab[4 * B + 4 * len(pieces):].view(B, 2)
     cb = torch.empty((B, chunk_size), dtype=torch.float32, device=dev)
     cd = torch.empty((B, chunk_size), dtype=torch.float32, device=dev)
     lib, st = _lib.lib(), _lib.stream_ptr(dev)
@@ -542,7 +557,8 @@
                 _lib.check(lib.bt_split_chunks_batch(_lib.stream_ptr(dev), spect.data_ptr(), d_rows[4 * i:].data_ptr(), nb,
                                                      chunk_size, chunks.data_ptr()))
                 if isinstance(model, BeatThis) and not _model_hooked(model):
-                    model._run(chunks, 0, 2, out=(cb[i: i + nb], cd[i: i + nb]), prec=prec, checks=checks)
+                    model._run(chunks, 0, 2, out=(cb[i: i + nb], cd[i: i + nb]), prec=prec, checks=checks,
+                               live=d_live[i: i + nb])
                 else:
                     r = model(chunks)
                     cb[i: i + nb], cd[i: i + nb] = r["beat"], r["downbeat"]
diff --git a/beat_this_amd/model/__init__.py b/beat_this_amd/model/__init__.py
--- a/beat_this_amd/model/__init__.py
+++ b/beat_this_amd/model/__init__.py
@@ -345,7 +345,7 @@
             return _lib.PREC_HALF
         return _lib.PREC_F32X3 if self.fp32_split_gemms and not _lib.lib().bt_half_is_bf16() else _lib.PREC_F32
 
-    def _run(self, x: torch.Tensor, first: int, last: int, out=None, prec=None, checks=None):
+    def _run(self, x: torch.Tensor, first: int, last: int, out=None, prec=None, checks=None, live=None):
         if x.dim() != 3:
             raise ValueError(f"expected a (batch, time, features) input, got {tuple(x.shape)}")
         _lib.require_gpu(x, "stage input")
@@ -354,7 +354,7 @@
             empty = torch.empty((x.shape[0], x.shape[1]), dtype=torch.float32, device=x.device)
             return (empty, empty.clone()) if last == 2 else torch.empty((x.shape[0], x.shape[1], D), dtype=torch.float32, device=x.device)
         prec = self._precision() if prec is None else prec
-        return self.engine(frontend_only=last == 0).forward_stages(x, prec, first, last, logits_out=out, checks=checks)
+        return self.engine(frontend_only=last == 0).forward_stages(x, prec, first, last, logits_out=out, checks=checks, live=live)
 
     def _run_unit(self, x: torch.Tensor, kind: str, index: int):
         _lib.require_gpu(x, "sub-module input")
diff --git a/beat_this_amd/pack.py b/beat_this_amd/pack.py
--- a/beat_this_amd/pack.py
+++ b/beat_this_amd/pack.py
@@ -400,9 +400,14 @@
     def forward(self, spect: torch.Tensor, prec: int):
         return self.forward_stages(spect, prec, 0, 2)
 
-    def forward_stages(self, spect: torch.Tensor, prec: int, first: int, last: int, logits_out=None, checks=None):
+    def forward_stages(self, spect: torch.Tensor, prec: int, first: int, last: int, logits_out=None, checks=None, live=None):
         _lib.require_gpu(spect, "stage input")
         B, T, M = spect.shape
+        if live is not None:
+            if first != 0 or last != 2:
+                raise ValueError("live row ranges go with a whole forward (stages 0..2)")
+            if live.dtype != torch.int32 or tuple(live.shape) != (B, 2) or not live.is_contiguous() or live.device != spect.device:
+                raise ValueError("live: a contiguous int32 (batch, 2) tensor on the input's device")
         D = self.packed.desc.transformer_dim
         if M != (128 if first == 0 else D):
             raise ValueError(f"expected {128 if first == 0 else D} input features, got {M}")
@@ -424,8 +429,12 @@
         else:
             out = torch.empty((B, T, D), dtype=torch.float32, device=self.device)
         with torch.cuda.device(self.device):
-            _lib.check(_lib.lib().bt_forward_stages(self._h, _lib.stream_ptr(self.device), prec, first, last, x.data_ptr(), B, T,
-                                                    ws.data_ptr(), ws.numel(), _lib.ptr(out), _lib.ptr(beat), _lib.ptr(down)))
+            if live is not None:
+                _lib.check(_lib.lib().bt_forward_live(self._h, _lib.stream_ptr(self.device), prec, x.data_ptr(), B, T, ws.data_ptr(),
+                                                      ws.numel(), beat.data_ptr(), down.data_ptr(), live.data_ptr()))
+            else:
+                _lib.check(_lib.lib().bt_forward_stages(self._h, _lib.stream_ptr(self.device), prec, first, last, x.data_ptr(), B, T,
+                                                        ws.data_ptr(), ws.numel(), _lib.ptr(out), _lib.ptr(beat), _lib.ptr(down)))
             if prec == _lib.PREC_F32X3:
                 flag = ws[:4].view(torch.int32)
                 if checks is not None:
@@ -436,7 +445,7 @@
                     checks.append((host, ev))
                 elif int(flag.item()) != 0:
                     self._count_fallback()
-                    return self.forward_stages(spect, _lib.PREC_F32, first, last, logits_out=logits_out)
+                    return self.forward_stages(spect, _lib.PREC_F32, first, last, logits_out=logits_out, live=live)
         return (beat, down) if last == 2 else out
 
     def forward_unit(self, x: torch.Tensor, prec: int, unit: int, index: int, out_shape) -> torch.Tensor:
diff --git a/include/beat_this_amd.h b/include/beat_this_amd.h
--- a/include/beat_this_amd.h
+++ b/include/beat_this_amd.h
@@ -98,6 +98,9 @@
 int bt_forward(bt_engine* e, void* stream, int prec, const float* d_spect, int B, int T, void* d_ws,
                size_t ws_bytes, float* d_beat, float* d_downbeat);
 
+int bt_forward_live(bt_engine* e, void* stream, int prec, const float* d_spect, int B, int T, void* d_ws, size_t ws_bytes,
+                    float* d_beat, float* d_downbeat, const int32_t* d_live);
+
 int bt_forward_stages(bt_engine* e, void* stream, int prec, int first, int last, const float* d_in, int B, int T, void* d_ws,
                       size_t ws_bytes, float* d_out, float* d_beat, float* d_downbeat);
 
@@ -273,6 +276,8 @@
 int bt_gemm3(void* stream, const bt_gemm3_args* a);
 int bt_attn_frag_blocks(int L);
 int bt_attention_frag(void* stream, const bt_attn_frag_args* a);
+int bt_gemm3_live(void* stream, const bt_gemm3_args* a, const int32_t* d_live, int live_T);
+int bt_attention_frag_live(void* stream, const bt_attn_frag_args* a, const int32_t* d_live);
 int bt_qkv_front(void* stream, int prec, const bt_pair_weights* w, const float* d_rope, const float* d_x, int B, int T, int F,
                  void* d_q, void* d_k, void* d_v, float* d_gates, int nbp);
 int bt_ff_fused(void* stream, int prec, const bt_pair_weights* w, float* d_x, int64_t M);
```

After: 64020, median of 6. About the same (+0.3%).
